# wwang2/CoarseGrainingVAE

Measured on NVIDIA B200. Metric: conformations/s (fwd+bwd train step), higher is better.
Workload: dtype f32

## Files before the change

coarsegrainingvae_b200/_lib.py:

```python
import ctypes
import os
import re

_HERE = os.path.dirname(os.path.abspath(__file__))
LIB_PATH = os.path.join(_HERE, "libcgvae_sm100.so")
HEADER_PATH = os.path.join(_HERE, "..", "include", "cgvae_b200.h")

_lib = None

_P = ctypes.c_void_p
_I64 = ctypes.c_int64
_INT = ctypes.c_int
_F32 = ctypes.c_float
_SZ = ctypes.c_size_t

SIGNATURES = {
    "cgvae_abi_version": (_INT, []),
    "cgvae_last_error": (ctypes.c_char_p, []),
    "cgvae_launch_count": (ctypes.c_ulonglong, []),
    "cgvae_set_error_flags": (_INT, [_INT, _P]),
    "cgvae_radius_graph_ws_bytes": (_SZ, [_I64, _I64]),
    "cgvae_radius_graph_count": (_INT, [_P, _I64, _P, _I64, _F32, _INT, _INT, _P, _P, _SZ, _P]),
    "cgvae_radius_graph_fill": (_INT, [_P, _I64, _P, _I64, _F32, _INT, _INT, _P, _P, _P, _SZ, _P]),
    "cgvae_exclusive_scan": (_INT, [_P, _I64, _P, _P]),
    "cgvae_edge_orientation": (_INT, [_P, _I64, _P, _P]),
    "cgvae_csr_count": (_INT, [_P, _I64, _P, _INT, _I64, _I64, _P, _P, _P]),
    "cgvae_scan_i32": (_INT, [_P, _I64, _P, _P]),
    "cgvae_csr_fill": (_INT, [_P, _I64, _P, _INT, _I64, _I64, _P, _P, _P, _P, _P, _P, _P, _P]),
    "cgvae_segment_count": (_INT, [_P, _I64, _I64, _P, _P]),
    "cgvae_segment_rank": (_INT, [_P, _I64, _I64, _P, _P, _P, _P, _P, _P]),
    "cgvae_edge_geometry": (_INT, [_P, _P, _P, _P, _P, _I64, _I64, _P, _INT, _INT, _F32, _P, _P, _P, _P, _P]),
    "cgvae_gemm": (_INT, [_INT, _P, _I64, _P, _I64, _P, _I64, _I64, _I64, _I64, _P, _INT, _P, _P, _INT, _P, _P, _SZ, _P, _INT, _P]),
    "cgvae_dense_pair_fwd": (_INT, [_P, _I64, _P, _I64, _I64, _I64, _I64, _I64, _P, _P, _P]),
    "cgvae_colsum": (_INT, [_P, _I64, _I64, _I64, _P, _P]),
    "cgvae_wgrad_grouped": (_INT, [_P, _INT, _P]),
    "cgvae_message_fwd": (_INT, [_INT, _P, _P, _P, _P, _P, _P, _P, _P, _P, _I64, _I64, _INT, _INT, _INT, _P, _P, _INT,
                                 _P, _P, _P, _P]),
    "cgvae_message_bwd_ws_bytes": (_SZ, [_INT, _INT, _INT, _I64]),
    "cgvae_message_bwd": (_INT, [_INT, _P, _P, _P, _P, _P, _P, _P, _P, _P, _P, _P, _I64, _I64, _INT, _INT, _INT, _P, _P,
                                 _INT, _INT, _P, _P, _P, _P, _P, _SZ, _P]),
    "cgvae_msg_tiles_batches_cap": (_I64, [_I64, _I64, _I64, _INT]),
    "cgvae_msg_tiles_rec_bytes": (_SZ, []),
    "cgvae_msg_tiles_build": (_INT, [_P, _P, _P, _I64, _I64, _I64, _P, _P, _INT, _INT, _P, _P, _P, _P, _I64, _P]),
    "cgvae_message_tc_ws_bytes": (_SZ, [_INT, _INT, _I64, _INT]),
    "cgvae_message_tc_fwd": (_INT, [_INT, _P, _P, _P, _P, _P, _P, _I64, _INT, _P, _P, _I64, _INT, _INT, _P, _P, _INT, _P, _P, _P,
                                    _P, _SZ, _P]),
    "cgvae_message9_fwd": (_INT, [_P, _P, _P, _P, _P, _P, _P, _P, _P, _P, _P, _I64, _INT, _INT, _INT, _INT, _P, _P, _P, _P, _P]),
    "cgvae_message9_bwd": (_INT, [_P, _P, _P, _P, _P, _P, _P, _P, _P, _P, _P, _P, _P, _P, _I64, _I64, _INT, _INT, _INT, _INT,
                                  _P, _P, _P, _P, _P, _P, _P, _P, _P, _P, _P]),
    "cgvae_update_norm_fwd": (_INT, [_P, _P, _I64, _INT, _P, _P]),
    "cgvae_update_combine_fwd": (_INT, [_P, _P, _P, _P, _P, _I64, _INT, _INT, _P, _P, _P]),
    "cgvae_update_combine_bwd": (_INT, [_P, _P, _P, _P, _P, _I64, _INT, _P, _P, _P, _P]),
    "cgvae_update_norm_bwd": (_INT, [_P, _P, _P, _P, _I64, _INT, _INT, _P, _P, _P]),
    "cgvae_update_combine_bwd_ld": (_INT, [_P, _P, _P, _P, _P, _I64, _INT, _P, _P, _P, _I64, _P]),
    "cgvae_update_norm_bwd_ld": (_INT, [_P, _P, _P, _P, _I64, _INT, _INT, _P, _P, _I64, _P]),
    "cgvae_segment_reduce_fwd": (_INT, [_P, _P, _P, _I64, _I64, _INT, _P, _P]),
    "cgvae_segment_reduce_bwd": (_INT, [_P, _P, _P, _I64, _I64, _INT, _P, _P]),
    "cgvae_gather_rows": (_INT, [_P, _P, _I64, _I64, _I64, _P, _P]),
    "cgvae_lift_fwd": (_INT, [_P, _P, _P, _P, _P, _P, _P, _I64, _I64, _INT, _INT, _P, _P]),
    "cgvae_lift_bwd": (_INT, [_P, _P, _P, _P, _P, _P, _I64, _I64, _INT, _INT, _P, _P]),
    "cgvae_adam_ws_bytes": (_SZ, []),
    "cgvae_adam_clip_step": (_INT, [_P, _P, _P, _P, _I64, _F32, _F32, _F32, _F32, _F32, _F32, _P, _P, _P, _F32, _F32, _P,
                                    _P, _SZ, _P]),
    "cgvae_bond_graph": (_INT, [_P, _P, _I64, _F32, _P, _P]),
    "cgvae_sample_quality": (_INT, [_P, _P, _P, _P, _I64, _I64, _F32, _P, _P, _P]),
    "cgvae_set_pdl": (_INT, [_INT]),
    "cgvae_set_matmul_precision": (_INT, [_INT]),
    "cgvae_get_matmul_precision": (_INT, []),
    "cgvae_register_const_range": (_INT, [_P, _SZ]),
    "cgvae_grad_sumsq": (_INT, [_P, _I64, _P, _P, _SZ, _P]),
    "cgvae_adam_apply": (_INT, [_P, _P, _P, _P, _I64, _F32, _F32, _F32, _F32, _F32, _F32, _P, _P, _INT, _F32, _F32, _P, _P, _SZ, _P]),
    "cgvae_dihedral_loss_fwd": (_INT, [_P, _P, _P, _I64, _P, _P, _P, _P, _P, _SZ, _P]),
    "cgvae_dihedral_loss_bwd": (_INT, [_P, _P, _P, _P, _I64, _I64, _P, _P, _P, _P]),
    "cgvae_pin_mask": (_INT, [_P, _I64, _P, _I64, _P, _SZ, _P]),
    "cgvae_vae_latent_fwd": (_INT, [_P, _P, _P, _I64, _P, _P, _P]),
    "cgvae_vae_latent_bwd": (_INT, [_P, _P, _P, _P, _I64, _P, _P, _P]),
    "cgvae_std_logvar_fwd": (_INT, [_P, _I64, _F32, _P, _P]),
    "cgvae_std_logvar_bwd": (_INT, [_P, _P, _I64, _F32, _P, _P]),
    "cgvae_loss_ws_bytes": (_SZ, []),
    "cgvae_loss_fwd": (_INT, [_P, _P, _I64, _P, _P, _P, _P, _P, _P, _I64, _INT, _P, _F32, _F32, _P, _P, _SZ, _P]),
    "cgvae_loss_bwd": (_INT, [_P, _P, _P, _I64, _P, _P, _P, _P, _P, _P, _I64, _INT, _P, _F32, _F32, _P, _P, _P, _P, _P, _P]),
    "cgvae_fill": (_INT, [_P, _I64, _F32, _P]),
    "cgvae_vec_to_planar": (_INT, [_P, _I64, _INT, _P, _P]),
    "cgvae_vec_from_planar": (_INT, [_P, _I64, _INT, _P, _P]),
}


def header_symbols():
    with open(HEADER_PATH) as fh:
        text = fh.read()
    text = re.sub(r"/\*.*?\*/", "", text, flags=re.S)
    return sorted(set(re.findall(r"\b(cgvae_[a-z0-9_]+)\s*\(", text)))


def load():
    global _lib
    if _lib is not None:
        return _lib
    if not os.path.exists(LIB_PATH):
        raise RuntimeError(
            "libcgvae_sm100.so not built (%s): run `python -m coarsegrainingvae_b200.build`; "
            "there is no CPU or PyTorch fallback" % LIB_PATH)
    lib = ctypes.CDLL(LIB_PATH)
    for name, (res, args) in SIGNATURES.items():
        fn = getattr(lib, name)
        fn.restype = res
        fn.argtypes = args
    if lib.cgvae_abi_version() != 1:
        raise RuntimeError("libcgvae_sm100.so ABI version mismatch")
    _lib = lib
    return lib


def last_error():
    return load().cgvae_last_error().decode("utf-8", "replace")


def launch_count():
    return int(load().cgvae_launch_count())


def check(rc, what):
    if rc != 0:
        raise RuntimeError("%s failed (code %d): %s" % (what, rc, last_error()))
```

coarsegrainingvae_b200/csrc/gemm_stream.cu:

```cuda
#include "common.cuh"
#include <cooperative_groups.h>
#include <cuda.h>
#include <algorithm>
#include <vector>

namespace cgvae {

struct StreamEpilogue {
  const float* bias;
  int act;
  float* z_out;
  const float* z_in;
  int dact;
  const float* add;
  float* C2;
  int n_split;
  int64_t ldc2;
};

__device__ __forceinline__ float stream_epilogue(const StreamEpilogue& ep, float v, int64_t m, int64_t n, int64_t ldc) {
  if (ep.bias) v += ep.bias[n];
  if (ep.z_out) ep.z_out[m * ldc + n] = v;
  v = act_fwd(ep.act, v);
  if (ep.z_in) v *= act_bwd(ep.dact, ep.z_in[m * ldc + n]);
  if (ep.add) v += ep.add[m * ldc + n];
  return v;
}

__host__ __device__ constexpr int wtr_count(int n, int off) { return (off >= 1 && n % 2 == 0) ? wtr_count(n / 2, off / 2) : n; }
__host__ __device__ constexpr int wtr_dupmask(int n, int off) { return (off >= 1 && n % 2 == 0) ? wtr_dupmask(n / 2, off / 2) : (off >= 1 ? 2 * off - 1 : 0); }

template <int N, int OFF>
__device__ __forceinline__ void wtr_step(float* v, int lane, int& base) {
  if constexpr (OFF >= 1 && (N % 2 == 0)) {
    constexpr int H = N / 2;
    const bool up = (lane & OFF) != 0;
#pragma unroll
    for (int i = 0; i < H; ++i) {
      const float send = up ? v[i] : v[i + H];
      const float keep = up ? v[i + H] : v[i];
      v[i] = keep + __shfl_xor_sync(0xffffffffu, send, OFF);
    }
    if (up) base += H;
    wtr_step<H, OFF / 2>(v, lane, base);
  } else if constexpr (OFF >= 1) {
#pragma unroll
    for (int i = 0; i < N; ++i) {
#pragma unroll
      for (int o = OFF; o >= 1; o >>= 1) v[i] += __shfl_xor_sync(0xffffffffu, v[i], o);
    }
  }
}

__device__ __forceinline__ uint32_t sm_u32(const void* p) { return (uint32_t)__cvta_generic_to_shared(p); }
__device__ __forceinline__ void bar_init(uint64_t* bar, uint32_t count) {
  asm volatile("mbarrier.init.shared::cta.b64 [%0], %1;" ::"r"(sm_u32(bar)), "r"(count));
}
__device__ __forceinline__ void bar_fence_init() { asm volatile("fence.mbarrier_init.release.cluster;" ::: "memory"); }
__device__ __forceinline__ void bar_expect_tx(uint64_t* bar, uint32_t bytes) {
  asm volatile("mbarrier.arrive.expect_tx.shared::cta.b64 _, [%0], %1;" ::"r"(sm_u32(bar)), "r"(bytes) : "memory");
}
__device__ __forceinline__ void bar_wait(uint64_t* bar, uint32_t parity) {
  for (uint32_t spin = 0; spin < (1u << 26); ++spin) {
    uint32_t done;
    asm volatile(
        "{\n"
        ".reg .pred p;\n"
        "mbarrier.try_wait.parity.shared::cta.b64 p, [%1], %2;\n"
        "selp.u32 %0, 1, 0, p;\n"
        "}\n"
        : "=r"(done)
        : "r"(sm_u32(bar)), "r"(parity)
        : "memory");
    if (done) return;
  }
  asm volatile("trap;");
}
__device__ __forceinline__ bool elect_lane() {
  uint32_t pred = 0;
  asm volatile(
      "{\n"
      ".reg .pred p;\n"
      "elect.sync _|p, 0xffffffff;\n"
      "selp.u32 %0, 1, 0, p;\n"
      "}\n"
      : "=r"(pred));
  return pred != 0;
}
__device__ __forceinline__ void bulk_g2s(void* dst, const void* src, uint32_t bytes, uint64_t* bar) {
  asm volatile("cp.async.bulk.shared::cluster.global.mbarrier::complete_tx::bytes [%0], [%1], %2, [%3];" ::"r"(sm_u32(dst)),
               "l"(src), "r"(bytes), "r"(sm_u32(bar))
               : "memory");
}
__device__ __forceinline__ void tma_2d_g2s(void* dst, const CUtensorMap* map, int c0, int c1, uint64_t* bar) {
  asm volatile("cp.async.bulk.tensor.2d.shared::cluster.global.mbarrier::complete_tx::bytes [%0], [%1, {%2, %3}], [%4];" ::"r"(
                   sm_u32(dst)),
               "l"(reinterpret_cast<uint64_t>(map)), "r"(c0), "r"(c1), "r"(sm_u32(bar))
               : "memory");
}

constexpr uint32_t kBulkPiece = 32768;

template <int MR, int RW>
__global__ void __launch_bounds__(MR > 16 ? 256 : 512) gemm_nt_stream_kernel(
    const float* __restrict__ X, int64_t ldx, const float* __restrict__ W, int64_t ldw, float* __restrict__ C, int64_t ldc,
    int M, int N, int K, int rows_per_cta, StreamEpilogue ep, int w_const) {
  if (!w_const) CGVAE_KERNEL_PROLOGUE();
  extern __shared__ __align__(128) float smem[];
  constexpr int NV = RW * MR;
  float* Xs = smem;
  float* Ws = smem + (size_t)MR * K;
  uint64_t* bar = reinterpret_cast<uint64_t*>(Ws + (size_t)rows_per_cta * K);
  const int tid = threadIdx.x, lane = tid & 31, warp = tid >> 5, nwarps = blockDim.x >> 5;
  const int row0 = blockIdx.x * rows_per_cta;
  const int rows = min(rows_per_cta, N - row0);

  if (tid == 0) {
    bar_init(bar, 1);
    bar_fence_init();
  }
  for (int idx = tid; idx < (MR - M) * (K / 4); idx += blockDim.x)
    reinterpret_cast<float4*>(Xs + (size_t)M * K)[idx] = make_float4(0.f, 0.f, 0.f, 0.f);
  __syncthreads();
  if (warp == 0 && elect_lane()) {
    const uint32_t row_bytes = (uint32_t)K * 4u;
    bar_expect_tx(bar, (uint32_t)(M + rows) * row_bytes);
    if (ldw == K) {
      const char* src = reinterpret_cast<const char*>(W + (int64_t)row0 * ldw);
      char* dst = reinterpret_cast<char*>(Ws);
      for (uint32_t off = 0, total = (uint32_t)rows * row_bytes; off < total; off += kBulkPiece)
        bulk_g2s(dst + off, src + off, min(kBulkPiece, total - off), bar);
    } else {
      for (int r = 0; r < rows; ++r) bulk_g2s(Ws + (size_t)r * K, W + (int64_t)(row0 + r) * ldw, row_bytes, bar);
    }
    if (w_const) pdl_wait();
    if (ldx == K) {
      const char* src = reinterpret_cast<const char*>(X);
      char* dst = reinterpret_cast<char*>(Xs);
      for (uint32_t off = 0, total = (uint32_t)M * row_bytes; off < total; off += kBulkPiece)
        bulk_g2s(dst + off, src + off, min(kBulkPiece, total - off), bar);
    } else {
      for (int m = 0; m < M; ++m) bulk_g2s(Xs + (size_t)m * K, X + (int64_t)m * ldx, row_bytes, bar);
    }
  }
  if (w_const) CGVAE_KERNEL_PROLOGUE();
  bar_wait(bar, 0);

  const int nchunks = (K + 127) / 128;
  for (int t0 = warp * RW; t0 < rows; t0 += nwarps * RW) {
    float acc[NV];
#pragma unroll
    for (int i = 0; i < NV; ++i) acc[i] = 0.f;
    for (int c = 0; c < nchunks; ++c) {
      const int k = c * 128 + lane * 4;
      if (k < K) {
        float4 w[RW];
#pragma unroll
        for (int r = 0; r < RW; ++r)
          w[r] = (t0 + r < rows) ? *reinterpret_cast<const float4*>(Ws + (size_t)(t0 + r) * K + k) : make_float4(0.f, 0.f, 0.f, 0.f);
#pragma unroll
        for (int m = 0; m < MR; ++m) {
          const float4 xv = *reinterpret_cast<const float4*>(Xs + (size_t)m * K + k);
#pragma unroll
          for (int r = 0; r < RW; ++r) {
            float a = acc[r * MR + m];
            a = fmaf(w[r].x, xv.x, a);
            a = fmaf(w[r].y, xv.y, a);
            a = fmaf(w[r].z, xv.z, a);
            a = fmaf(w[r].w, xv.w, a);
            acc[r * MR + m] = a;
          }
        }
      }
    }
    int base = 0;
    wtr_step<NV, 16>(acc, lane, base);
    constexpr int CNT = wtr_count(NV, 16);
    constexpr int DUP = wtr_dupmask(NV, 16);
    if ((lane & DUP) == 0) {
#pragma unroll
      for (int i = 0; i < CNT; ++i) {
        const int idx = base + i;
        const int r = idx / MR, m = idx % MR;
        const int n = row0 + t0 + r;
        if (m < M && t0 + r < rows) {
          if (ep.C2 != nullptr && n >= ep.n_split) ep.C2[(int64_t)m * ep.ldc2 + (n - ep.n_split)] = acc[i];
          else C[(int64_t)m * ldc + n] = stream_epilogue(ep, acc[i], m, n, ldc);
        }
      }
    }
  }
}

constexpr int NN_MAXBOX = 8;

template <int VEC> struct VecT;
template <> struct VecT<2> { using type = float2; };
template <> struct VecT<4> { using type = float4; };

template <int MR, int VEC, int NW>
__global__ void __launch_bounds__(NW * 32) gemm_nn_stream_kernel(
    const __grid_constant__ CUtensorMap wmap, const float* __restrict__ G, int64_t ldg, float* __restrict__ C, int64_t ldc,
    int M, int N, int K, int k_per_cta, int box_rows, StreamEpilogue ep, int w_const) {
  if (!w_const) CGVAE_KERNEL_PROLOGUE();
  namespace cg = cooperative_groups;
  using vec_t = typename VecT<VEC>::type;
  constexpr int COLS = 32 * VEC;
  extern __shared__ __align__(128) float smem[];
  const int nbox = (k_per_cta + box_rows - 1) / box_rows;
  float* Wt = smem;
  float* red = smem;
  const size_t wt_floats = (size_t)max(nbox * box_rows, NW * MR) * COLS;
  float* part = smem + wt_floats;
  float* Gt = part + MR * COLS;
  uint64_t* bars = reinterpret_cast<uint64_t*>(Gt + (size_t)k_per_cta * MR);
  const int tid = threadIdx.x, lane = tid & 31, warp = tid >> 5;
  const int col0 = blockIdx.x * COLS;
  const int kbeg = blockIdx.z * k_per_cta;
  const int cnt = max(0, min(K, kbeg + k_per_cta) - kbeg);

  if (tid == 0) {
    for (int b = 0; b < nbox; ++b) bar_init(bars + b, 1);
    bar_fence_init();
  }
  __syncwarp();
  if (warp == 0 && elect_lane()) {
    for (int b = 0; b < nbox; ++b) {
      if (b * box_rows < cnt) {
        bar_expect_tx(bars + b, (uint32_t)box_rows * COLS * 4u);
        tma_2d_g2s(Wt + (size_t)b * box_rows * COLS, &wmap, col0, kbeg + b * box_rows, bars + b);
      }
    }
  }
  if (w_const) CGVAE_KERNEL_PROLOGUE();
  for (int idx = tid; idx < MR * cnt; idx += NW * 32) {
    const int m = idx / cnt, j = idx - m * cnt;
    Gt[j * MR + m] = (m < M) ? __ldg(G + (int64_t)m * ldg + kbeg + j) : 0.f;
  }
  __syncthreads();

  float acc[MR][VEC];
#pragma unroll
  for (int m = 0; m < MR; ++m)
#pragma unroll
    for (int v = 0; v < VEC; ++v) acc[m][v] = 0.f;

  for (int b = 0; b * box_rows < cnt; ++b) {
    bar_wait(bars + b, 0);
    const int jend = min(cnt, (b + 1) * box_rows);
#pragma unroll 2
    for (int j = b * box_rows + warp; j < jend; j += NW) {
      const vec_t t = *reinterpret_cast<const vec_t*>(Wt + (size_t)j * COLS + lane * VEC);
      float w[VEC];
      if constexpr (VEC == 2) { w[0] = t.x; w[1] = t.y; }
      if constexpr (VEC == 4) { w[0] = t.x; w[1] = t.y; w[2] = t.z; w[3] = t.w; }
      const float* g = Gt + j * MR;
#pragma unroll
      for (int m4 = 0; m4 < MR / 4; ++m4) {
        const float4 g4 = *reinterpret_cast<const float4*>(g + 4 * m4);
#pragma unroll
        for (int v = 0; v < VEC; ++v) {
          acc[4 * m4 + 0][v] = fmaf(g4.x, w[v], acc[4 * m4 + 0][v]);
          acc[4 * m4 + 1][v] = fmaf(g4.y, w[v], acc[4 * m4 + 1][v]);
          acc[4 * m4 + 2][v] = fmaf(g4.z, w[v], acc[4 * m4 + 2][v]);
          acc[4 * m4 + 3][v] = fmaf(g4.w, w[v], acc[4 * m4 + 3][v]);
        }
      }
    }
  }
  __syncthreads();
#pragma unroll
  for (int m = 0; m < MR; ++m)
#pragma unroll
    for (int v = 0; v < VEC; ++v) red[(warp * MR + m) * COLS + lane * VEC + v] = acc[m][v];
  __syncthreads();
  for (int o = tid; o < MR * COLS; o += NW * 32) {
    float s = 0.f;
#pragma unroll
    for (int wv = 0; wv < NW; ++wv) s += red[wv * MR * COLS + o];
    part[o] = s;
  }
  cg::cluster_group cluster = cg::this_cluster();
  cluster.sync();
  const int S = (int)cluster.num_blocks(), rank = (int)cluster.block_rank();
  for (int o = tid; o < MR * COLS; o += NW * 32) {
    const int m = o / COLS, c = o - m * COLS;
    if (m % S != rank) continue;
    const int n = col0 + c;
    if (m < M && n < N) {
      float s = 0.f;
      for (int z = 0; z < S; ++z) s += *cluster.map_shared_rank(part + o, z);
      C[(int64_t)m * ldc + n] = stream_epilogue(ep, s, m, n, ldc);
    }
  }
  cluster.sync();
}

typedef CUresult (*EncodeTiledFn)(CUtensorMap*, CUtensorMapDataType, cuuint32_t, void*, const cuuint64_t*, const cuuint64_t*,
                                  const cuuint32_t*, const cuuint32_t*, CUtensorMapInterleave, CUtensorMapSwizzle,
                                  CUtensorMapL2promotion, CUtensorMapFloatOOBfill);

static EncodeTiledFn encode_tiled_fn() {
  static EncodeTiledFn fn = [] {
    void* p = nullptr;
    cudaDriverEntryPointQueryResult q;
    if (cudaGetDriverEntryPoint("cuTensorMapEncodeTiled", &p, cudaEnableDefault, &q) != cudaSuccess || q != cudaDriverEntryPointSuccess) {
      (void)cudaGetLastError();
      p = nullptr;
    }
    return reinterpret_cast<EncodeTiledFn>(p);
  }();
  return fn;
}

constexpr size_t kMaxStreamSmem = 220 * 1024;

struct ConstRange {
  uintptr_t begin, end;
};
static std::vector<ConstRange> g_const_ranges;

bool weights_are_constant(const void* p, size_t bytes) {
  if (!pdl_enabled() || g_const_ranges.empty()) return false;
  const uintptr_t a = reinterpret_cast<uintptr_t>(p);
  auto it = std::upper_bound(g_const_ranges.begin(), g_const_ranges.end(), a,
                             [](uintptr_t v, const ConstRange& r) { return v < r.begin; });
  if (it == g_const_ranges.begin()) return false;
  --it;
  return a >= it->begin && a + bytes <= it->end;
}

template <int MR, int RW>
static bool launch_nt(const float* X, int64_t ldx, const float* W, int64_t ldw, float* C, int64_t ldc, int M, int N, int K,
                      const StreamEpilogue& ep, cudaStream_t st) {
  const int w_const = weights_are_constant(W, sizeof(float) * ((size_t)(N - 1) * (size_t)ldw + (size_t)K)) ? 1 : 0;
  int rpc = (int)ceil_div(ceil_div(N, kNumSM), RW) * RW;
  const size_t smem = sizeof(float) * ((size_t)MR * K + (size_t)rpc * K) + 16;
  if (smem > kMaxStreamSmem) return false;
  static size_t attr_bytes = 0;
  if (smem > attr_bytes) {
    if (cudaFuncSetAttribute(gemm_nt_stream_kernel<MR, RW>, cudaFuncAttributeMaxDynamicSharedMemorySize, (int)kMaxStreamSmem) != cudaSuccess) {
      (void)cudaGetLastError();
      return false;
    }
    attr_bytes = kMaxStreamSmem;
  }
  const int tasks = rpc / RW;
  const int nwarps = tasks <= 2 ? 2 : (tasks <= 4 ? 4 : ((tasks <= 8 || MR > 16) ? 8 : 16));
  launch_kernel(gemm_nt_stream_kernel<MR, RW>, dim3((unsigned)ceil_div(N, rpc)), dim3(nwarps * 32), smem, st, X, ldx, W, ldw, C, ldc, M,
                N, K, rpc, ep, w_const);
  return true;
}

template <int MR, int VEC, int NW>
static bool launch_nn(const float* G, int64_t ldg, const float* W, int64_t ldw, float* C, int64_t ldc, int M, int N, int K,
                      const StreamEpilogue& ep, cudaStream_t st) {
  const int w_const = weights_are_constant(W, sizeof(float) * ((size_t)(K - 1) * (size_t)ldw + (size_t)N)) ? 1 : 0;
  constexpr int COLS = 32 * VEC;
  EncodeTiledFn encode = encode_tiled_fn();
  if (encode == nullptr) return false;
  const int blocks = (int)ceil_div(N, COLS);
  int S = (int)std::min<int64_t>(8, std::max<int64_t>(1, kNumSM / blocks));
  S = (int)std::min<int64_t>(S, std::max<int64_t>(1, K / NW));
  while (S & (S - 1)) S &= S - 1;
  int k_per_cta = (int)ceil_div(K, S);
  S = (int)ceil_div(K, k_per_cta);
  const int nbox = (int)ceil_div(k_per_cta, 256);
  if (nbox > NN_MAXBOX) return false;
  const int box_rows = (int)ceil_div(k_per_cta, nbox);
  const size_t wt_floats = (size_t)std::max(nbox * box_rows, NW * MR) * COLS;
  const size_t smem = sizeof(float) * (wt_floats + (size_t)MR * COLS + (size_t)k_per_cta * MR) + 8 * NN_MAXBOX;
  if (smem > kMaxStreamSmem) return false;
  CUtensorMap map;
  const cuuint64_t gdim[2] = {(cuuint64_t)N, (cuuint64_t)K};
  const cuuint64_t gstride[1] = {(cuuint64_t)ldw * 4};
  const cuuint32_t box[2] = {(cuuint32_t)COLS, (cuuint32_t)box_rows};
  const cuuint32_t estride[2] = {1, 1};
  if (encode(&map, CU_TENSOR_MAP_DATA_TYPE_FLOAT32, 2, const_cast<float*>(W), gdim, gstride, box, estride, CU_TENSOR_MAP_INTERLEAVE_NONE,
             CU_TENSOR_MAP_SWIZZLE_NONE, CU_TENSOR_MAP_L2_PROMOTION_L2_256B, CU_TENSOR_MAP_FLOAT_OOB_FILL_NONE) != CUDA_SUCCESS)
    return false;
  static size_t attr_bytes = 0;
  if (smem > attr_bytes) {
    if (cudaFuncSetAttribute(gemm_nn_stream_kernel<MR, VEC, NW>, cudaFuncAttributeMaxDynamicSharedMemorySize, (int)kMaxStreamSmem) != cudaSuccess) {
      (void)cudaGetLastError();
      return false;
    }
    attr_bytes = kMaxStreamSmem;
  }
  cudaLaunchConfig_t cfg = {};
  cfg.gridDim = dim3((unsigned)blocks, 1, (unsigned)S);
  cfg.blockDim = dim3(NW * 32);
  cfg.dynamicSmemBytes = smem;
  cfg.stream = st;
  cudaLaunchAttribute attr[2];
  attr[0].id = cudaLaunchAttributeClusterDimension;
  attr[0].val.clusterDim.x = 1;
  attr[0].val.clusterDim.y = 1;
  attr[0].val.clusterDim.z = (unsigned)S;
  attr[1].id = cudaLaunchAttributeProgrammaticStreamSerialization;
  attr[1].val.programmaticStreamSerializationAllowed = 1;
  cfg.attrs = attr;
  cfg.numAttrs = pdl_enabled() ? 2 : 1;
  (void)cudaLaunchKernelEx(&cfg, gemm_nn_stream_kernel<MR, VEC, NW>, map, G, ldg, C, ldc, M, N, K, k_per_cta, box_rows, ep, w_const);
  return true;
}

int launch_gemm_stream(int form, const float* A, int64_t lda, const float* B, int64_t ldb, float* C, int64_t ldc, int64_t M,
                       int64_t N, int64_t K, const float* bias, int act, float* z_out, const float* z_in, int dact,
                       const float* add, cudaStream_t st) {
  static const bool enabled = [] { const char* e = getenv("CGVAE_STREAM_GEMM"); return !(e && e[0] == '0'); }();
  if (!enabled || M > 48 || M < 1 || form == CGVAE_GEMM_TN) return 0;
  if (N * K < 64 * 64 || N >= (1 << 24) || K >= (1 << 24)) return 0;
  const StreamEpilogue ep{bias, act, z_out, z_in, dact, add, nullptr, 0, 0};
  const int m = (int)M, n = (int)N, k = (int)K;
  if (form == CGVAE_GEMM_NT) {
    if (K % 4 != 0 || K < 128 || lda % 4 != 0 || ldb % 4 != 0 || !aligned16(A) || !aligned16(B)) return 0;
    if (M <= 12) return launch_nt<12, 4>(A, lda, B, ldb, C, ldc, m, n, k, ep, st);
    if (M <= 16) return launch_nt<16, 4>(A, lda, B, ldb, C, ldc, m, n, k, ep, st);
    if (M <= 36) return launch_nt<36, 2>(A, lda, B, ldb, C, ldc, m, n, k, ep, st);
    return launch_nt<48, 2>(A, lda, B, ldb, C, ldc, m, n, k, ep, st);
  }
  if (K < 64 || N < 64 || ldb % 4 != 0 || !aligned16(B)) return 0;
  const bool wide = ceil_div(N, 64) * 2 > kNumSM;
  if (M <= 12) return wide ? launch_nn<12, 4, 16>(A, lda, B, ldb, C, ldc, m, n, k, ep, st) : launch_nn<12, 2, 16>(A, lda, B, ldb, C, ldc, m, n, k, ep, st);
  if (M <= 16) return wide ? launch_nn<16, 4, 16>(A, lda, B, ldb, C, ldc, m, n, k, ep, st) : launch_nn<16, 2, 16>(A, lda, B, ldb, C, ldc, m, n, k, ep, st);
  static const bool nn_wide_rows = [] { const char* e = getenv("CGVAE_STREAM_NN_ROWS48"); return e && e[0] == '1'; }();
  if (!nn_wide_rows) return 0;
  if (M <= 36) return launch_nn<36, 2, 8>(A, lda, B, ldb, C, ldc, m, n, k, ep, st);
  return launch_nn<48, 2, 8>(A, lda, B, ldb, C, ldc, m, n, k, ep, st);
}

int launch_dense_pair_stream(const float* X, int64_t ldx, const float* W, int64_t ldw, float* C1, int64_t ldc1, float* C2,
                             int64_t ldc2, int64_t M, int64_t N1, int64_t N2, int64_t K, cudaStream_t st) {
  static const bool enabled = [] { const char* e = getenv("CGVAE_STREAM_GEMM"); return !(e && e[0] == '0'); }();
  if (!enabled || M > 48 || M < 1 || N1 + N2 >= (1 << 24) || K >= (1 << 24)) return 0;
  if (K % 4 != 0 || K < 128 || ldx % 4 != 0 || ldw % 4 != 0 || !aligned16(X) || !aligned16(W)) return 0;
  const StreamEpilogue ep{nullptr, 0, nullptr, nullptr, 0, nullptr, C2, (int)N1, ldc2};
  const int m = (int)M, n = (int)(N1 + N2), k = (int)K;
  if (M <= 12) return launch_nt<12, 4>(X, ldx, W, ldw, C1, ldc1, m, n, k, ep, st);
  if (M <= 16) return launch_nt<16, 4>(X, ldx, W, ldw, C1, ldc1, m, n, k, ep, st);
  if (M <= 36) return launch_nt<36, 2>(X, ldx, W, ldw, C1, ldc1, m, n, k, ep, st);
  return launch_nt<48, 2>(X, ldx, W, ldw, C1, ldc1, m, n, k, ep, st);
}

}

extern "C" {

int cgvae_register_const_range(const void* p, size_t bytes) {
  using namespace cgvae;
  if (p == nullptr || bytes == 0) {
    g_const_ranges.clear();
    return 0;
  }
  ConstRange r{reinterpret_cast<uintptr_t>(p), reinterpret_cast<uintptr_t>(p) + bytes};
  std::vector<ConstRange> out;
  out.reserve(g_const_ranges.size() + 1);
  for (const ConstRange& q : g_const_ranges) {
    if (q.end < r.begin || q.begin > r.end) out.push_back(q);
    else {
      r.begin = std::min(r.begin, q.begin);
      r.end = std::max(r.end, q.end);
    }
  }
  out.push_back(r);
  std::sort(out.begin(), out.end(), [](const ConstRange& x, const ConstRange& y) { return x.begin < y.begin; });
  g_const_ranges.swap(out);
  return 0;
}

}
```

coarsegrainingvae_b200/csrc/nodewise.cu:

```cuda
#include "common.cuh"

namespace cgvae {

__global__ void __launch_bounds__(256) update_norm_fwd_kernel(const float* __restrict__ s, const float* __restrict__ Vv, int64_t N,
                                                              int F, float* __restrict__ x) {
  CGVAE_KERNEL_PROLOGUE();
  const int64_t idx = (int64_t)blockIdx.x * blockDim.x + threadIdx.x;
  if (idx >= N * F) return;
  const int64_t n = idx / F;
  const int f = (int)(idx % F);
  const float* p = Vv + n * 3 * F + f;
  const float a = __fadd_rn(__fmul_rn(p[0], p[0]), 1e-10f);
  const float b = __fadd_rn(__fmul_rn(p[F], p[F]), 1e-10f);
  const float c = __fadd_rn(__fmul_rn(p[2 * (int64_t)F], p[2 * (int64_t)F]), 1e-10f);
  x[n * 2 * F + f] = s[idx];
  x[n * 2 * F + F + f] = __fsqrt_rn(__fadd_rn(__fadd_rn(a, b), c));
}

__global__ void __launch_bounds__(256) update_combine_fwd_kernel(const float* __restrict__ s, const float* __restrict__ v,
                                                                 const float* __restrict__ Uv, const float* __restrict__ Vv,
                                                                 const float* __restrict__ q, int64_t N, int F, int residual,
                                                                 float* __restrict__ s_out, float* __restrict__ v_out) {
  CGVAE_KERNEL_PROLOGUE();
  const int64_t idx = (int64_t)blockIdx.x * blockDim.x + threadIdx.x;
  if (idx >= N * F) return;
  const int64_t n = idx / F;
  const int f = (int)(idx % F);
  const int64_t o = n * 3 * F + f;
  const float a_vv = q[o], a_sv = q[o + F], a_ss = q[o + 2 * (int64_t)F];
  float inner = 0.f;
#pragma unroll
  for (int c = 0; c < 3; ++c) {
    const float u = Uv[o + (int64_t)c * F], w = Vv[o + (int64_t)c * F];
    inner = fmaf(u, w, inner);
    v_out[o + (int64_t)c * F] = (residual ? v[o + (int64_t)c * F] : 0.f) + u * a_vv;
  }
  s_out[idx] = (residual ? s[idx] : 0.f) + (inner * a_sv + a_ss);
}

__global__ void __launch_bounds__(256) update_combine_bwd_kernel(const float* __restrict__ Uv, const float* __restrict__ Vv,
                                                                 const float* __restrict__ q, const float* __restrict__ g_s,
                                                                 const float* __restrict__ g_v, int64_t N, int F,
                                                                 float* __restrict__ gq, float* __restrict__ gUv,
                                                                 float* __restrict__ gVv, int64_t ldg) {
  CGVAE_KERNEL_PROLOGUE();
  const int64_t idx = (int64_t)blockIdx.x * blockDim.x + threadIdx.x;
  if (idx >= N * F) return;
  const int64_t n = idx / F;
  const int f = (int)(idx % F);
  const int64_t o = n * 3 * F + f;
  const int64_t og = n * 3 * ldg + f;
  const float a_vv = q[o], a_sv = q[o + F];
  const float gs = g_s[idx];
  float inner = 0.f, g_avv = 0.f;
  const float t = gs * a_sv;
#pragma unroll
  for (int c = 0; c < 3; ++c) {
    const float u = Uv[o + (int64_t)c * F], w = Vv[o + (int64_t)c * F], g = g_v[o + (int64_t)c * F];
    inner = fmaf(u, w, inner);
    g_avv = fmaf(g, u, g_avv);
    gUv[og + (int64_t)c * ldg] = g * a_vv + t * w;
    gVv[og + (int64_t)c * ldg] = t * u;
  }
  gq[o] = g_avv;
  gq[o + F] = gs * inner;
  gq[o + 2 * (int64_t)F] = gs;
}

__global__ void __launch_bounds__(256) update_norm_bwd_kernel(const float* __restrict__ x, const float* __restrict__ Vv,
                                                              const float* __restrict__ gx, const float* __restrict__ g_s,
                                                              int64_t N, int F, int residual, float* __restrict__ gs_in,
                                                              float* __restrict__ gVv, int64_t ldg) {
  CGVAE_KERNEL_PROLOGUE();
  const int64_t idx = (int64_t)blockIdx.x * blockDim.x + threadIdx.x;
  if (idx >= N * F) return;
  const int64_t n = idx / F;
  const int f = (int)(idx % F);
  gs_in[idx] = (residual ? g_s[idx] : 0.f) + gx[n * 2 * F + f];
  const float scale = gx[n * 2 * F + F + f] / x[n * 2 * F + F + f];
  const int64_t o = n * 3 * F + f, og = n * 3 * ldg + f;
#pragma unroll
  for (int c = 0; c < 3; ++c) gVv[og + (int64_t)c * ldg] = fmaf(scale, Vv[o + (int64_t)c * F], gVv[og + (int64_t)c * ldg]);
}

__global__ void __launch_bounds__(256) segment_reduce_fwd_kernel(const float* __restrict__ X, const int32_t* __restrict__ rowptr_b,
                                                                 const int32_t* __restrict__ atoms, int64_t W, int mean,
                                                                 float* __restrict__ out) {
  CGVAE_KERNEL_PROLOGUE();
  const int64_t b = blockIdx.x;
  const int64_t w = (int64_t)blockIdx.y * blockDim.x + threadIdx.x;
  if (w >= W) return;
  const int beg = rowptr_b[b], end = rowptr_b[b + 1];
  float acc = 0.f;
  for (int t = beg; t < end; ++t) acc += X[(int64_t)atoms[t] * W + w];
  if (mean) acc = acc / (float)max(end - beg, 1);
  out[b * W + w] = acc;
}
__global__ void __launch_bounds__(256) segment_reduce_bwd_kernel(const float* __restrict__ g_out, const int64_t* __restrict__ mapping,
                                                                 const int32_t* __restrict__ rowptr_b, int64_t W, int mean,
                                                                 float* __restrict__ g_X) {
  CGVAE_KERNEL_PROLOGUE();
  const int64_t a = blockIdx.x;
  const int64_t w = (int64_t)blockIdx.y * blockDim.x + threadIdx.x;
  if (w >= W) return;
  const int64_t b = mapping[a];
  float g = g_out[b * W + w];
  if (mean) g = g / (float)max(rowptr_b[b + 1] - rowptr_b[b], 1);
  g_X[a * W + w] = g;
}

__global__ void __launch_bounds__(256) gather_rows_kernel(const float* __restrict__ table, const int64_t* __restrict__ idx, int64_t W,
                                                          int64_t n_rows, float* __restrict__ out, int32_t* __restrict__ err) {
  CGVAE_KERNEL_PROLOGUE();
  const int64_t n = blockIdx.x;
  const int64_t w = (int64_t)blockIdx.y * blockDim.x + threadIdx.x;
  if (w >= W) return;
  const int64_t r = idx[n];
  if (n_rows > 0 && (r < 0 || r >= n_rows)) {
    if (w == 0) raise_flag(err, CGVAE_ERR_EMBED_INDEX);
    out[n * W + w] = __int_as_float(0x7fc00000);
    return;
  }
  out[n * W + w] = table[r * W + w];
}

__global__ void __launch_bounds__(128) lift_fwd_kernel(const float* __restrict__ V, const float* __restrict__ cg_xyz,
                                                       const int64_t* __restrict__ rank, const int32_t* __restrict__ rowptr_b,
                                                       const int32_t* __restrict__ atoms, const uint8_t* __restrict__ pin,
                                                       int64_t n_beads, int F, int mode, float* __restrict__ xyz_out,
                                                       int32_t* __restrict__ err) {
  CGVAE_KERNEL_PROLOGUE();
  const int lane = threadIdx.x & 31;
  const int64_t b = (int64_t)blockIdx.x * 4 + (threadIdx.x >> 5);
  if (b >= n_beads) return;
  const int beg = rowptr_b[b], end = rowptr_b[b + 1];
  const float* Vb = V + b * 3 * F;
  float mean[3] = {0.f, 0.f, 0.f};
  if (mode == 1) {
    for (int t = beg + lane; t < end; t += 32) {
      const int64_t ch = rank[atoms[t]];
      if (ch >= F) continue;
#pragma unroll
      for (int c = 0; c < 3; ++c) mean[c] += Vb[(int64_t)c * F + ch];
    }
    const float inv = 1.0f / (float)max(end - beg, 1);
#pragma unroll
    for (int c = 0; c < 3; ++c) mean[c] = warp_sum(mean[c]) * inv;
  }
  for (int t = beg + lane; t < end; t += 32) {
    const int a = atoms[t];
    const int64_t ch = rank[a];
    const bool pinned = (mode == 2) && pin != nullptr && pin[a] != 0;
    if (ch >= F) {
      raise_flag(err, CGVAE_ERR_LIFT_RANK);
#pragma unroll
      for (int c = 0; c < 3; ++c) xyz_out[(int64_t)a * 3 + c] = __int_as_float(0x7fc00000);
      continue;
    }
#pragma unroll
    for (int c = 0; c < 3; ++c) {
      const float rel = pinned ? 0.f : Vb[(int64_t)c * F + ch] - mean[c];
      xyz_out[(int64_t)a * 3 + c] = rel + cg_xyz[b * 3 + c];
    }
  }
}
__global__ void __launch_bounds__(128) lift_bwd_kernel(const float* __restrict__ g_xyz, const int64_t* __restrict__ rank,
                                                       const int32_t* __restrict__ rowptr_b, const int32_t* __restrict__ atoms,
                                                       const uint8_t* __restrict__ pin, int64_t n_beads, int F, int mode,
                                                       float* __restrict__ g_V) {
  CGVAE_KERNEL_PROLOGUE();
  const int lane = threadIdx.x & 31;
  const int64_t b = (int64_t)blockIdx.x * 4 + (threadIdx.x >> 5);
  if (b >= n_beads) return;
  const int beg = rowptr_b[b], end = rowptr_b[b + 1];
  float* gVb = g_V + b * 3 * F;
  float mean[3] = {0.f, 0.f, 0.f};
  if (mode == 1) {
    for (int t = beg + lane; t < end; t += 32) {
      const int a = atoms[t];
#pragma unroll
      for (int c = 0; c < 3; ++c) mean[c] += g_xyz[(int64_t)a * 3 + c];
    }
    const float inv = 1.0f / (float)max(end - beg, 1);
#pragma unroll
    for (int c = 0; c < 3; ++c) mean[c] = warp_sum(mean[c]) * inv;
  }
  for (int t = beg + lane; t < end; t += 32) {
    const int a = atoms[t];
    const int64_t ch = rank[a];
    const bool pinned = (mode == 2) && pin != nullptr && pin[a] != 0;
    if (ch >= F) continue;
#pragma unroll
    for (int c = 0; c < 3; ++c) gVb[(int64_t)c * F + ch] = pinned ? 0.f : g_xyz[(int64_t)a * 3 + c] - mean[c];
  }
}

__global__ void __launch_bounds__(256) pin_mask_kernel(const int64_t* __restrict__ idx, int64_t n_idx, const int64_t* __restrict__ n_live,
                                                       int64_t n_atoms, uint8_t* __restrict__ pin, int32_t* __restrict__ err) {
  CGVAE_KERNEL_PROLOGUE();
  const int64_t n = n_live ? min(*n_live, n_idx) : n_idx;
  const int64_t i = (int64_t)blockIdx.x * blockDim.x + threadIdx.x;
  if (i >= n || n <= 0) return;
  if (idx[n - 1] >= n_atoms) return;
  const int64_t a = idx[i];
  if (a < 0 || a >= n_atoms) {
    raise_flag(err, CGVAE_ERR_NODE_INDEX);
    return;
  }
  pin[a] = 1;
}

}

using namespace cgvae;

extern "C" {

int cgvae_pin_mask(const int64_t* idx, int64_t n_idx, const int64_t* n_live, int64_t n_atoms, uint8_t* pin, size_t pin_bytes,
                   cgvae_stream_t stream) {
  cudaStream_t st = (cudaStream_t)stream;
  if (n_atoms == 0) return 0;
  CGVAE_REQUIRE(pin && pin_bytes >= (size_t)n_atoms && pin_bytes % 4 == 0, "pin_mask: pin buffer must hold n_atoms bytes, padded to 4");
  CGVAE_ZERO(pin, pin_bytes, st);
  if (n_idx == 0) return 0;
  CGVAE_REQUIRE(idx, "pin_mask: null index list");
  launch_kernel(pin_mask_kernel, dim3((unsigned)ceil_div(n_idx, 256)), dim3(256), 0, st, idx, n_idx, n_live, n_atoms, pin, err_flags());
  return launched("pin_mask");
}

int cgvae_update_norm_fwd(const float* s, const float* Vv, int64_t N, int F, float* x, cgvae_stream_t stream) {
  if (N == 0) return 0;
  CGVAE_REQUIRE(s && Vv && x, "update_norm_fwd: null pointer");
  launch_kernel(update_norm_fwd_kernel, dim3((unsigned)ceil_div(N * F, 256)), dim3(256), 0, (cudaStream_t)stream, s, Vv, N, F, x);
  return launched("update_norm_fwd");
}
int cgvae_update_combine_fwd(const float* s, const float* v, const float* Uv, const float* Vv, const float* q, int64_t N, int F,
                             int residual, float* s_out, float* v_out, cgvae_stream_t stream) {
  if (N == 0) return 0;
  CGVAE_REQUIRE(Uv && Vv && q && s_out && v_out && (!residual || (s && v)), "update_combine_fwd: null pointer");
  launch_kernel(update_combine_fwd_kernel, dim3((unsigned)ceil_div(N * F, 256)), dim3(256), 0, (cudaStream_t)stream, s, v, Uv, Vv, q, N, F, residual, s_out,
                                                                                             v_out);
  return launched("update_combine_fwd");
}
int cgvae_update_combine_bwd(const float* Uv, const float* Vv, const float* q, const float* g_s, const float* g_v, int64_t N, int F,
                             float* gq, float* gUv, float* gVv, cgvae_stream_t stream) {
  if (N == 0) return 0;
  CGVAE_REQUIRE(Uv && Vv && q && g_s && g_v && gq && gUv && gVv, "update_combine_bwd: null pointer");
  launch_kernel(update_combine_bwd_kernel, dim3((unsigned)ceil_div(N * F, 256)), dim3(256), 0, (cudaStream_t)stream, Uv, Vv, q, g_s, g_v, N, F, gq, gUv, gVv, (int64_t)F);
  return launched("update_combine_bwd");
}
int cgvae_update_norm_bwd(const float* x, const float* Vv, const float* gx, const float* g_s, int64_t N, int F, int residual,
                          float* gs_in, float* gVv, cgvae_stream_t stream) {
  if (N == 0) return 0;
  CGVAE_REQUIRE(x && Vv && gx && gs_in && gVv && (!residual || g_s), "update_norm_bwd: null pointer");
  launch_kernel(update_norm_bwd_kernel, dim3((unsigned)ceil_div(N * F, 256)), dim3(256), 0, (cudaStream_t)stream, x, Vv, gx, g_s, N, F, residual, gs_in, gVv, (int64_t)F);
  return launched("update_norm_bwd");
}

int cgvae_update_combine_bwd_ld(const float* Uv, const float* Vv, const float* q, const float* g_s, const float* g_v, int64_t N, int F,
                                float* gq, float* gUv, float* gVv, int64_t ldg, cgvae_stream_t stream) {
  if (N == 0) return 0;
  CGVAE_REQUIRE(Uv && Vv && q && g_s && g_v && gq && gUv && gVv && ldg >= F, "update_combine_bwd_ld: bad arguments");
  launch_kernel(update_combine_bwd_kernel, dim3((unsigned)ceil_div(N * F, 256)), dim3(256), 0, (cudaStream_t)stream, Uv, Vv, q, g_s, g_v, N, F, gq,
                gUv, gVv, ldg);
  return launched("update_combine_bwd");
}
int cgvae_update_norm_bwd_ld(const float* x, const float* Vv, const float* gx, const float* g_s, int64_t N, int F, int residual,
                             float* gs_in, float* gVv, int64_t ldg, cgvae_stream_t stream) {
  if (N == 0) return 0;
  CGVAE_REQUIRE(x && Vv && gx && gs_in && gVv && (!residual || g_s) && ldg >= F, "update_norm_bwd_ld: bad arguments");
  launch_kernel(update_norm_bwd_kernel, dim3((unsigned)ceil_div(N * F, 256)), dim3(256), 0, (cudaStream_t)stream, x, Vv, gx, g_s, N, F, residual,
                gs_in, gVv, ldg);
  return launched("update_norm_bwd");
}

int cgvae_segment_reduce_fwd(const float* X, const int32_t* rowptr_b, const int32_t* atoms, int64_t n_beads, int64_t W, int mean,
                             float* out, cgvae_stream_t stream) {
  if (n_beads == 0 || W == 0) return 0;
  CGVAE_REQUIRE(X && rowptr_b && atoms && out, "segment_reduce_fwd: null pointer");
  dim3 grid((unsigned)n_beads, (unsigned)ceil_div(W, 256));
  launch_kernel(segment_reduce_fwd_kernel, dim3(grid), dim3(256), 0, (cudaStream_t)stream, X, rowptr_b, atoms, W, mean, out);
  return launched("segment_reduce_fwd");
}
int cgvae_segment_reduce_bwd(const float* g_out, const int64_t* mapping, const int32_t* rowptr_b, int64_t N, int64_t W, int mean,
                             float* g_X, cgvae_stream_t stream) {
  if (N == 0 || W == 0) return 0;
  CGVAE_REQUIRE(g_out && mapping && rowptr_b && g_X, "segment_reduce_bwd: null pointer");
  dim3 grid((unsigned)N, (unsigned)ceil_div(W, 256));
  launch_kernel(segment_reduce_bwd_kernel, dim3(grid), dim3(256), 0, (cudaStream_t)stream, g_out, mapping, rowptr_b, W, mean, g_X);
  return launched("segment_reduce_bwd");
}
int cgvae_gather_rows(const float* table, const int64_t* idx, int64_t N, int64_t W, int64_t n_rows, float* out,
                      cgvae_stream_t stream) {
  if (N == 0 || W == 0) return 0;
  CGVAE_REQUIRE(table && idx && out, "gather_rows: null pointer");
  dim3 grid((unsigned)N, (unsigned)ceil_div(W, 256));
  launch_kernel(gather_rows_kernel, dim3(grid), dim3(256), 0, (cudaStream_t)stream, table, idx, W, n_rows, out, err_flags());
  return launched("gather_rows");
}

int cgvae_lift_fwd(const float* V, const float* cg_xyz, const int64_t* mapping, const int64_t* rank, const int32_t* rowptr_b,
                   const int32_t* atoms, const uint8_t* pin, int64_t N, int64_t n_beads, int F, int mode, float* xyz_out,
                   cgvae_stream_t stream) {
  (void)mapping;
  if (N == 0 || n_beads == 0) return 0;
  CGVAE_REQUIRE(V && cg_xyz && rank && rowptr_b && atoms && xyz_out, "lift_fwd: null pointer");
  CGVAE_REQUIRE(mode >= 0 && mode <= 2, "lift_fwd: bad mode %d", mode);
  launch_kernel(lift_fwd_kernel, dim3((unsigned)ceil_div(n_beads, 4)), dim3(128), 0, (cudaStream_t)stream, V, cg_xyz, rank, rowptr_b, atoms, pin, n_beads, F,
                                                                                   mode, xyz_out, err_flags());
  return launched("lift_fwd");
}
int cgvae_lift_bwd(const float* g_xyz, const int64_t* mapping, const int64_t* rank, const int32_t* rowptr_b, const int32_t* atoms,
                   const uint8_t* pin, int64_t N, int64_t n_beads, int F, int mode, float* g_V, cgvae_stream_t stream) {
  (void)mapping;
  cudaStream_t st = (cudaStream_t)stream;
  if (n_beads == 0) return 0;
  CGVAE_REQUIRE(g_xyz && rank && rowptr_b && atoms && g_V, "lift_bwd: null pointer");
  CGVAE_ZERO(g_V, sizeof(float) * (size_t)n_beads * 3 * (size_t)F, st);
  if (N == 0) return 0;
  launch_kernel(lift_bwd_kernel, dim3((unsigned)ceil_div(n_beads, 4)), dim3(128), 0, st, g_xyz, rank, rowptr_b, atoms, pin, n_beads, F, mode, g_V);
  return launched("lift_bwd");
}

}
```

coarsegrainingvae_b200/functions.py:

```python
import torch
from torch.autograd import Function
from torch.autograd.function import once_differentiable

from . import ops

SWISH = 1


def _phi_forward(s, W1, b1, W2, b2, act=SWISH):
    a1, z1 = ops.linear_fwd(s, W1, b1, act, save_pre=True)
    phi = ops.linear_fwd(a1, W2, b2, 0)
    return a1, z1, phi


def _phi_backward(g_phi2d, s, a1, z1, W1, b1, W2, b2, add_to_gs, act=SWISH):
    fork = ops.Fork(g_phi2d.device, enabled=not ops.deferring(g_phi2d.shape[0]))
    gz1 = ops.linear_bwd_input(g_phi2d, W2, z_in=z1, dact=act)
    with fork.branch():
        gW2 = ops.linear_bwd_weight(g_phi2d, a1, W2)
        gb2 = ops.colsum(g_phi2d, b2)
    fork.sync()
    gs = ops.linear_bwd_input(gz1, W1, add=add_to_gs)
    with fork.branch():
        gW1 = ops.linear_bwd_weight(gz1, s, W1)
        gb1 = ops.colsum(gz1, b1)
    fork.join()
    return gs, gW1, gb1, gW2, gb2


class MLP2(Function):

    @staticmethod
    def forward(ctx, act, x, W1, b1, W2, b2):
        x = x.contiguous()
        a1, z1, y = _phi_forward(x, W1, b1, W2, b2, act)
        ctx.act = act
        ctx.save_for_backward(x, a1, z1, W1, b1, W2, b2)
        return y

    @staticmethod
    @once_differentiable
    def backward(ctx, gy):
        x, a1, z1, W1, b1, W2, b2 = ctx.saved_tensors
        gx, gW1, gb1, gW2, gb2 = _phi_backward(gy.contiguous(), x, a1, z1, W1, b1, W2, b2, None, ctx.act)
        return None, gx, gW1, gb1, gW2, gb2


class LinearFn(Function):

    @staticmethod
    def forward(ctx, x, W, b):
        x = x.contiguous()
        ctx.save_for_backward(x, W, b)
        return ops.linear_fwd(x, W, b, 0)

    @staticmethod
    @once_differentiable
    def backward(ctx, gy):
        x, W, b = ctx.saved_tensors
        gy = gy.contiguous()
        fork = ops.Fork(gy.device, enabled=not ops.deferring(gy.shape[0]))
        gx = ops.linear_bwd_input(gy, W)
        with fork.branch():
            gW = ops.linear_bwd_weight(gy, x, W)
            gb = ops.colsum(gy, b) if b is not None else None
        fork.join()
        return gx, gW, gb


class MessageBlock(Function):

    @staticmethod
    def forward(ctx, geom, n_split, mode, act, s, v, res_s, res_v, W1, b1, W2, b2, Wf, bf):
        s = s.contiguous()
        a1, z1, phi = _phi_forward(s, W1, b1, W2, b2, act)
        N, F = s.shape
        phi3 = phi.view(N, n_split, F)
        if mode == "self":
            rs, rv = s, v
        elif mode == "other":
            rs, rv = res_s, res_v
        else:
            rs, rv = None, None
        out_s, out_v, q = ops.message_fwd(n_split, phi3, v, v if n_split == 4 else None, geom, Wf, bf, rs, rv,
                                          want_q=(n_split == 4 and v is not None))
        ctx.geom, ctx.n_split, ctx.mode, ctx.act = geom, n_split, mode, act
        ctx.v_none = v is None
        ctx.res_v_none = res_v is None
        ctx.save_for_backward(s, v, a1, z1, phi3, q, W1, b1, W2, b2, Wf, bf)
        return out_s, out_v

    @staticmethod
    @once_differentiable
    def backward(ctx, g_s, g_v):
        s, v, a1, z1, phi3, q, W1, b1, W2, b2, Wf, bf = ctx.saved_tensors
        g_s, g_v = g_s.contiguous(), g_v.contiguous()
        n_split, mode = ctx.n_split, ctx.mode
        residual = mode == "self"
        g_phi, g_v_send, dWf, dbf = ops.message_bwd(n_split, phi3, v, v if n_split == 4 else None, q, ctx.geom, Wf, bf,
                                                    g_s, g_v, residual and not ctx.v_none)
        N, F = s.shape
        gs, gW1, gb1, gW2, gb2 = _phi_backward(g_phi.view(N, n_split * F), s, a1, z1, W1, b1, W2, b2,
                                               g_s if residual else None, ctx.act)
        gv = None if ctx.v_none else g_v_send
        g_res_s = g_s if mode == "other" else None
        g_res_v = g_v if (mode == "other" and not ctx.res_v_none) else None
        return None, None, None, None, gs, gv, g_res_s, g_res_v, gW1, gb1, gW2, gb2, dWf, dbf


class Message9Block(Function):

    @staticmethod
    def forward(ctx, geom, residual, act, s, sbar, v, vbar, W1, b1, W2, b2, Wf, bf):
        s, sbar, v, vbar = s.contiguous(), sbar.contiguous(), v.contiguous(), vbar.contiguous()
        a1, z1, phi = _phi_forward(s, W1, b1, W2, b2, act)
        N, F = s.shape
        phi3 = phi.view(N, 9, F)
        outs = ops.message9_fwd(phi3, s, sbar, v, vbar, geom, Wf, bf, residual)
        ctx.geom, ctx.residual, ctx.act = geom, residual, act
        ctx.save_for_backward(s, sbar, v, vbar, a1, z1, phi3, W1, b1, W2, b2, Wf, bf)
        return tuple(outs)

    @staticmethod
    @once_differentiable
    def backward(ctx, g_s, g_sbar, g_v, g_vbar):
        s, sbar, v, vbar, a1, z1, phi3, W1, b1, W2, b2, Wf, bf = ctx.saved_tensors
        gi_s, gi_sbar, gi_v, gi_vbar, g_phi, dWf, dbf = ops.message9_bwd(
            phi3, s, sbar, v, vbar, ctx.geom, Wf, bf, ctx.residual,
            g_s.contiguous(), g_sbar.contiguous(), g_v.contiguous(), g_vbar.contiguous())
        N, F = s.shape
        gs, gW1, gb1, gW2, gb2 = _phi_backward(g_phi.view(N, 9 * F), s, a1, z1, W1, b1, W2, b2, gi_s, ctx.act)
        return None, None, None, gs, gi_sbar, gi_v, gi_vbar, gW1, gb1, gW2, gb2, dWf, dbf


class UpdateBlockFn(Function):

    @staticmethod
    def forward(ctx, residual, act, s, v, U, V, A0, c0, A1, c1):
        s, v = s.contiguous(), v.contiguous()
        N, F = s.shape
        v2 = v.view(3 * N, F)
        Uv, Vv = ops.linear_pair_fwd(v2, U, V)
        Uv, Vv = Uv.view(N, 3, F), Vv.view(N, 3, F)
        x = ops.update_norm_fwd(s, Vv)
        h, z = ops.linear_fwd(x, A0, c0, act, save_pre=True)
        q = ops.linear_fwd(h, A1, c1, 0).view(N, 3, F)
        s_out, v_out = ops.update_combine_fwd(s, v, Uv, Vv, q, residual)
        ctx.residual, ctx.act = residual, act
        ctx.save_for_backward(v, Uv, Vv, x, h, z, q, U, V, A0, c0, A1, c1)
        return s_out, v_out

    @staticmethod
    @once_differentiable
    def backward(ctx, g_s, g_v):
        v, Uv, Vv, x, h, z, q, U, V, A0, c0, A1, c1 = ctx.saved_tensors
        g_s, g_v = g_s.contiguous(), g_v.contiguous()
        N, _, F = v.shape
        pair = (U.is_cuda and U.is_contiguous() and V.is_contiguous() and U.shape == V.shape
                and V.data_ptr() == U.data_ptr() + 4 * U.numel()
                and U.untyped_storage().data_ptr() == V.untyped_storage().data_ptr())
        gq, gUv, gVv = ops.update_combine_bwd(Uv, Vv, q, g_s, g_v, cat=pair)
        gq2 = gq.view(N, 3 * F)
        v2 = v.view(3 * N, F)
        if pair:
            gUV2 = gUv.as_strided((3 * N, 2 * F), (2 * F, 1))
            gUv2, gVv2 = gUV2[:, :F], gUV2[:, F:]
        else:
            gUv2, gVv2 = gUv.view(3 * N, F), gVv.view(3 * N, F)
        fork = ops.Fork(g_s.device, enabled=not ops.deferring(3 * N))
        gz = ops.linear_bwd_input(gq2, A1, z_in=z, dact=ctx.act)
        with fork.branch():
            gA1 = ops.linear_bwd_weight(gq2, h, A1)
            gc1 = ops.colsum(gq2, c1)
            if not pair:
                gU = ops.linear_bwd_weight(gUv2, v2, U)
        fork.sync()
        gx = ops.linear_bwd_input(gz, A0)
        with fork.branch():
            gA0 = ops.linear_bwd_weight(gz, x, A0)
            gc0 = ops.colsum(gz, c0)
        gs_in = ops.update_norm_bwd(x, Vv, gx, g_s, gVv, ctx.residual)
        fork.sync()
        if pair:
            UV = U.as_strided((2 * F, U.shape[1]), (U.shape[1], 1))
            gv_in = ops.linear_bwd_input(gUV2, UV, add=g_v.view(3 * N, F) if ctx.residual else None).view(N, 3, F)
        else:
            gv_in = ops.linear_bwd_input(gUv2, U, add=g_v.view(3 * N, F) if ctx.residual else None)
            gv_in = ops.linear_bwd_input(gVv2, V, add=gv_in).view(N, 3, F)
        with fork.branch():
            if pair:
                gUVw = ops.linear_bwd_weight(gUV2, v2, U, shape=(2 * F, U.shape[1]))
                gU, gV = gUVw[:F], gUVw[F:]
            else:
                gV = ops.linear_bwd_weight(gVv2, v2, V)
        fork.join()
        return None, None, gs_in, gv_in, gU, gV, gA0, gc0, gA1, gc1


class SegmentReduce(Function):

    @staticmethod
    def forward(ctx, seg, mean, X):
        ctx.seg, ctx.mean = seg, mean
        return ops.segment_reduce_fwd(X.contiguous(), seg, mean)

    @staticmethod
    @once_differentiable
    def backward(ctx, g):
        return None, None, ops.segment_reduce_bwd(g.contiguous(), ctx.seg, ctx.mean)


class EmbeddingLookup(Function):

    @staticmethod
    def forward(ctx, table, idx, padding_idx):
        idx = idx.to(torch.int64).contiguous()
        ctx.padding_idx = padding_idx
        ctx.n_rows = table.shape[0]
        ctx.save_for_backward(idx, table)
        return ops.gather_rows(table, idx)

    @staticmethod
    @once_differentiable
    def backward(ctx, g):
        idx, table = ctx.saved_tensors
        seg = ops.build_segments(idx, ctx.n_rows)
        gt = ops.segment_reduce_fwd(g.contiguous(), seg, False, param=table)
        if ctx.padding_idx is not None:
            gt[ctx.padding_idx].zero_()
        return gt, None, None


class Lift(Function):

    @staticmethod
    def forward(ctx, seg, mode, pin, V, cg_xyz):
        ctx.seg, ctx.mode, ctx.pin, ctx.F = seg, mode, pin, V.shape[-1]
        return ops.lift_fwd(V.contiguous(), cg_xyz, seg, mode, pin)

    @staticmethod
    @once_differentiable
    def backward(ctx, g):
        return None, None, None, ops.lift_bwd(g.contiguous(), ctx.seg, ctx.F, ctx.mode, ctx.pin), None


class VAELatent(Function):

    @staticmethod
    def forward(ctx, mu, logvar, eps):
        z, sigma = ops.vae_latent_fwd(mu, logvar, eps)
        ctx.save_for_backward(eps, sigma)
        return z, sigma

    @staticmethod
    @once_differentiable
    def backward(ctx, g_z, g_sigma):
        eps, sigma = ctx.saved_tensors
        g_mu, g_logvar = ops.vae_latent_bwd(g_z.contiguous() if g_z is not None else None,
                                            g_sigma.contiguous() if g_sigma is not None else None, eps, sigma)
        return g_mu, g_logvar, None


class StdLogvar(Function):

    @staticmethod
    def forward(ctx, x, c):
        y = ops.std_logvar_fwd(x, c)
        ctx.c = c
        ctx.save_for_backward(y)
        return y

    @staticmethod
    @once_differentiable
    def backward(ctx, gy):
        (y,) = ctx.saved_tensors
        return ops.std_logvar_bwd(gy.contiguous(), y, ctx.c), None


class TrainingLoss(Function):

    @staticmethod
    def forward(ctx, bond_graph, beta, gamma, norms, xyz, xyz_rec, mu, sigma, pmu, pstd):
        xyz, xyz_rec = xyz.contiguous(), xyz_rec.contiguous()
        if mu is not None:
            mu, sigma = mu.contiguous(), sigma.contiguous()
        if pmu is not None:
            pmu, pstd = pmu.contiguous(), pstd.contiguous()
        out4 = ops.loss_fwd(xyz, xyz_rec, bond_graph, mu, sigma, pmu, pstd, norms, beta, gamma)
        ctx.bond_graph, ctx.beta, ctx.gamma, ctx.norms = bond_graph, beta, gamma, norms
        ctx.has = (mu is not None, pmu is not None)
        ctx.save_for_backward(xyz, xyz_rec, *([mu, sigma] if mu is not None else []), *([pmu, pstd] if pmu is not None else []))
        comps = out4.detach()
        ctx.mark_non_differentiable(comps)
        return out4.narrow(0, 0, 1).reshape(()), comps

    @staticmethod
    @once_differentiable
    def backward(ctx, g_loss, _g_comps):
        saved = list(ctx.saved_tensors)
        xyz, xyz_rec = saved[0], saved[1]
        mu = sigma = pmu = pstd = None
        k = 2
        if ctx.has[0]:
            mu, sigma = saved[k], saved[k + 1]
            k += 2
        if ctx.has[1]:
            pmu, pstd = saved[k], saved[k + 1]
        g = g_loss.reshape(1).contiguous()
        g_rec, g_mu, g_sigma, g_pmu, g_pstd = ops.loss_bwd(g, xyz, xyz_rec, ctx.bond_graph, mu, sigma, pmu, pstd, ctx.norms,
                                                           ctx.beta, ctx.gamma)
        return None, None, None, None, None, g_rec, g_mu, g_sigma, g_pmu, g_pstd


class DihedralLoss(Function):

    @staticmethod
    def forward(ctx, xyz, xyz_rec, idx, count, norm):
        n_atoms = xyz_rec.shape[0]
        idx = idx.to(torch.int64).contiguous()
        out, contrib = ops.dihedral_loss_fwd(xyz.contiguous(), xyz_rec.contiguous(), idx, count, norm)
        D = idx.shape[0]
        pairs = torch.stack([idx.reshape(-1), torch.arange(4 * D, dtype=torch.int64, device=idx.device)], 1)
        ctx.graph = ops.build_graph(pairs, n_atoms, n_send=max(4 * D, 1))
        ctx.n_atoms, ctx.count, ctx.norm = n_atoms, count, norm
        ctx.save_for_backward(contrib)
        return out.reshape(())

    @staticmethod
    @once_differentiable
    def backward(ctx, g):
        (contrib,) = ctx.saved_tensors
        g_rec = ops.dihedral_loss_bwd(g.reshape(1).contiguous(), contrib, ctx.graph, ctx.n_atoms, ctx.count, ctx.norm)
        return None, g_rec, None, None, None
```

coarsegrainingvae_b200/ops.py:

```python
import contextlib as _contextlib

import numpy as np
import torch

from . import _lib

ACT_CODES = {None: 0, "none": 0, "linear": 0, "swish": 1, "ReLU": 2, "relu": 2, "Tanh": 3, "tanh": 3}
GEMM_NT, GEMM_NN, GEMM_TN = 0, 1, 2


def _p(t):
    if t is None:
        return None
    return t.data_ptr()


_raw_stream = torch._C._cuda_getCurrentRawStream if hasattr(torch._C, "_cuda_getCurrentRawStream") else None


def _stream():
    if _raw_stream is not None:
        return _raw_stream(torch.cuda.current_device())
    return torch.cuda.current_stream().cuda_stream


def _need_cuda(*tensors):
    for t in tensors:
        if t is not None and not t.is_cuda:
            raise RuntimeError("coarsegrainingvae_b200 runs on CUDA tensors only (sm_100a kernels, no CPU fallback); "
                               "got a %s tensor" % t.device)


def _f32(t):
    if t.dtype != torch.float32:
        raise RuntimeError("expected float32, got %s" % t.dtype)
    return t.contiguous()


def launch_count():
    return _lib.launch_count()


VALIDATE = True
_ERR_FLAGS = {}
_ERR_TEXT = {1: "a bead holds more atoms than feature channels (cg_v[mapping, CG2atomChannel], cgvae.py:473)",
             2: "embedding index out of range (nn.Embedding, cgvae.py:273,380,591)",
             4: "CG_mapping entry outside [0, n_beads)",
             8: "edge-list entry outside [0, n_nodes)"}


def error_flags(device):
    idx = device.index if device.index is not None else torch.cuda.current_device()
    t = _ERR_FLAGS.get(idx)
    if t is None:
        t = torch.zeros(1, dtype=torch.int32, device=torch.device("cuda", idx))
        _ERR_FLAGS[idx] = t
        _lib.check(_lib.load().cgvae_set_error_flags(idx, t.data_ptr()), "set_error_flags")
    return t


def check_device_errors(device, force=False):
    if not (VALIDATE or force) or device.type != "cuda" or torch.cuda.is_current_stream_capturing():
        return
    t = error_flags(device)
    bits = int(t.item())
    if bits:
        t.zero_()
        raise IndexError("; ".join(msg for bit, msg in _ERR_TEXT.items() if bits & bit))


class KernelTimer(object):

    def __init__(self, names, keep_operands=False):
        self.names = set(names)
        self.records = {}
        self.keep_operands = keep_operands

    def begin(self, name):
        if name not in self.names:
            return None
        ev = torch.cuda.Event(enable_timing=True)
        ev.record(torch.cuda.current_stream())
        return ev

    def end(self, name, start, meta):
        if start is None:
            return
        ev = torch.cuda.Event(enable_timing=True)
        ev.record(torch.cuda.current_stream())
        self.records.setdefault(name, []).append((start, ev, meta))

    def summary(self):
        return {k: [(a.elapsed_time(b), m) for a, b, m in v] for k, v in self.records.items()}


TIMER = None

_SIDE_STREAMS = {}
FORK_ENABLED = True


class Fork(object):

    def __init__(self, device, enabled=True):
        self.enabled = enabled and FORK_ENABLED and device.type == "cuda"
        if not self.enabled:
            return
        idx = device.index if device.index is not None else torch.cuda.current_device()
        side = _SIDE_STREAMS.get(idx)
        if side is None:
            side = torch.cuda.Stream(device=idx)
            _SIDE_STREAMS[idx] = side
        self.side = side
        self.main = torch.cuda.current_stream(idx)
        self.sync()

    def sync(self):
        if self.enabled:
            ev = torch.cuda.Event()
            ev.record(self.main)
            self.side.wait_event(ev)

    def branch(self):
        if self.enabled:
            return torch.cuda.stream(self.side)
        import contextlib
        return contextlib.nullcontext()

    def join(self):
        if self.enabled:
            ev = torch.cuda.Event()
            ev.record(self.side)
            self.main.wait_event(ev)


GRAD_SINK = {}


def _has_sink(param):
    return (param is not None and bool(GRAD_SINK) and param.grad is None and GRAD_SINK.get(param.data_ptr()) is not None)


def _grad_out(param, shape):
    hit = GRAD_SINK.get(param.data_ptr()) if GRAD_SINK else None
    if hit is None or param.grad is not None:
        return torch.empty(shape, dtype=param.dtype, device=param.device)
    flat, off = hit
    n = 1
    for s in shape:
        n *= s
    return flat[off:off + n].view(shape)



class Graph(object):

    def __init__(self, n_recv, n_send, n_edges, rowptr, col, eid, rowptr_t, col_t, perm_t):
        self.n_recv, self.n_send, self.n_edges = int(n_recv), int(n_send), int(n_edges)
        self.rowptr, self.col, self.eid = rowptr, col, eid
        self.rowptr_t, self.col_t, self.perm_t = rowptr_t, col_t, perm_t


class Geometry(object):

    def __init__(self, graph, basis, unit, n_rbf, rb, cutoff):
        self.graph, self.basis, self.unit = graph, basis, unit
        self.n_rbf, self.rb, self.cutoff = int(n_rbf), int(rb), float(cutoff)


class Segments(object):

    def __init__(self, n_beads, mapping, rowptr, atoms, slot, rank):
        self.n_beads, self.mapping = int(n_beads), mapping
        self.rowptr, self.atoms, self.slot, self.rank = rowptr, atoms, slot, rank
        self.n = int(mapping.shape[0])


def rb_for(n_rbf):
    rb = ((n_rbf + 1 + 3) // 4) * 4
    if rb < 8:
        rb = 8
    if rb > 16:
        raise RuntimeError("n_rbf up to 15 supported (got %d)" % n_rbf)
    return rb


_COEF_CACHE = {}


def rbf_coefficients(n_rbf, cutoff, device):
    key = (int(n_rbf), float(cutoff), str(device))
    hit = _COEF_CACHE.get(key)
    if hit is None:
        n = torch.arange(1, n_rbf + 1).float()
        hit = (n * np.pi / cutoff).to(device)
        _COEF_CACHE[key] = hit
    return hit


def exclusive_scan(counts_i32, out_dtype=torch.int64):
    _need_cuda(counts_i32)
    lib = _lib.load()
    n = counts_i32.shape[0]
    out = torch.empty(n + 1, dtype=out_dtype, device=counts_i32.device)
    if out_dtype == torch.int64:
        _lib.check(lib.cgvae_exclusive_scan(_p(counts_i32), n, _p(out), _stream()), "exclusive_scan")
    else:
        _lib.check(lib.cgvae_scan_i32(_p(counts_i32), n, _p(out), _stream()), "scan_i32")
    return out


def radius_graph(xyz, cutoff, undirected=True, frame_ptr=None, use_cells=None, capacity=None, max_frame=None):
    _need_cuda(xyz)
    lib = _lib.load()
    xyz = _f32(xyz)
    n = xyz.shape[0]
    dev = xyz.device
    if frame_ptr is None:
        frame_ptr = torch.tensor([0, n], dtype=torch.int64, device=dev)
        max_frame = n
    else:
        frame_ptr = frame_ptr.to(device=dev, dtype=torch.int64).contiguous()
    n_frames = frame_ptr.shape[0] - 1
    if capacity is not None:
        if max_frame is None:
            raise ValueError("radius_graph(capacity=...) needs max_frame (atoms of the largest frame): no host read in static mode")
        worst = n_frames * max_frame * (max_frame - 1) // (2 if undirected else 1)
        if capacity < worst:
            raise ValueError("capacity %d below the worst case %d (%d frames of <= %d atoms)" % (capacity, worst, n_frames, max_frame))
    if use_cells is None:
        if max_frame is None:
            max_frame = int((frame_ptr[1:] - frame_ptr[:-1]).max().item()) if n_frames > 0 else 0
        use_cells = max_frame > 1024
    if n == 0:
        if capacity is not None:
            return torch.zeros((capacity, 2), dtype=torch.int64, device=dev), torch.zeros(1, dtype=torch.int64, device=dev)
        return torch.zeros((0, 2), dtype=torch.int64, device=dev)
    ws_bytes = int(lib.cgvae_radius_graph_ws_bytes(n, n_frames)) if use_cells else 0
    ws = torch.empty(max(ws_bytes, 16), dtype=torch.uint8, device=dev)
    deg = torch.empty(n, dtype=torch.int32, device=dev)
    st = _stream()
    _lib.check(lib.cgvae_radius_graph_count(_p(xyz), n, _p(frame_ptr), n_frames, float(np.float32(cutoff)), int(bool(undirected)),
                                            int(bool(use_cells)), _p(deg), _p(ws), ws_bytes, st), "radius_graph_count")
    rowptr = exclusive_scan(deg, torch.int64)
    if capacity is not None:
        pairs = torch.zeros((capacity, 2), dtype=torch.int64, device=dev)
        _lib.check(lib.cgvae_radius_graph_fill(_p(xyz), n, _p(frame_ptr), n_frames, float(np.float32(cutoff)), int(bool(undirected)),
                                               int(bool(use_cells)), _p(rowptr), _p(pairs), _p(ws), ws_bytes, st),
                   "radius_graph_fill")
        return pairs, rowptr[-1:].clone()
    n_edges = int(rowptr[-1].item())
    pairs = torch.empty((n_edges, 2), dtype=torch.int64, device=dev)
    if n_edges:
        _lib.check(lib.cgvae_radius_graph_fill(_p(xyz), n, _p(frame_ptr), n_frames, float(np.float32(cutoff)), int(bool(undirected)),
                                               int(bool(use_cells)), _p(rowptr), _p(pairs), _p(ws), ws_bytes, st),
                   "radius_graph_fill")
    return pairs


def edge_orientation(pairs):
    _need_cuda(pairs)
    lib = _lib.load()
    flags = torch.empty(2, dtype=torch.int32, device=pairs.device)
    pairs = pairs.contiguous()
    _lib.check(lib.cgvae_edge_orientation(_p(pairs), pairs.shape[0], _p(flags), _stream()), "edge_orientation")
    f = flags.tolist()
    return bool(f[0]), bool(f[1])


def build_graph(pairs, n_recv, n_send=None, symmetrize=False, n_edges_dev=None):
    _need_cuda(pairs)
    lib = _lib.load()
    if n_send is None:
        n_send = n_recv
    pairs = pairs.to(torch.int64).contiguous()
    E_in = pairs.shape[0]
    E = 2 * E_in if symmetrize else E_in
    dev = pairs.device
    st = _stream()
    sym = int(bool(symmetrize))
    error_flags(dev)
    deg_r = torch.empty(n_recv, dtype=torch.int32, device=dev)
    deg_s = torch.empty(n_send, dtype=torch.int32, device=dev)
    _lib.check(lib.cgvae_csr_count(_p(pairs), E_in, _p(n_edges_dev), sym, n_recv, n_send, _p(deg_r), _p(deg_s), st), "csr_count")
    rowptr = exclusive_scan(deg_r, torch.int32)
    rowptr_t = exclusive_scan(deg_s, torch.int32)
    col = torch.empty(E, dtype=torch.int32, device=dev)
    eid = torch.empty(E, dtype=torch.int32, device=dev)
    col_t = torch.empty(E, dtype=torch.int32, device=dev)
    perm_t = torch.empty(E, dtype=torch.int32, device=dev)
    scratch = torch.empty(n_recv + n_send + 2 * E + 4, dtype=torch.int32, device=dev)
    _lib.check(lib.cgvae_csr_fill(_p(pairs), E_in, _p(n_edges_dev), sym, n_recv, n_send, _p(rowptr), _p(rowptr_t), _p(scratch),
                                  _p(col), _p(eid), _p(col_t), _p(perm_t), st), "csr_fill")
    return Graph(n_recv, n_send, E, rowptr, col, eid, rowptr_t, col_t, perm_t)


def build_segments(mapping, n_beads):
    _need_cuda(mapping)
    lib = _lib.load()
    mapping = mapping.to(torch.int64).contiguous()
    n = mapping.shape[0]
    dev = mapping.device
    st = _stream()
    error_flags(dev)
    deg = torch.empty(n_beads, dtype=torch.int32, device=dev)
    _lib.check(lib.cgvae_segment_count(_p(mapping), n, n_beads, _p(deg), st), "segment_count")
    rowptr = exclusive_scan(deg, torch.int32)
    atoms = torch.empty(n, dtype=torch.int32, device=dev)
    slot = torch.empty(n, dtype=torch.int32, device=dev)
    rank = torch.empty(n, dtype=torch.int64, device=dev)
    scratch = torch.empty(n_beads + 4, dtype=torch.int32, device=dev)
    _lib.check(lib.cgvae_segment_rank(_p(mapping), n, n_beads, _p(rowptr), _p(scratch), _p(atoms), _p(slot), _p(rank), st),
               "segment_rank")
    return Segments(n_beads, mapping, rowptr, atoms, slot, rank)


def contraction_graph(seg):
    dev = seg.mapping.device
    n = seg.n
    rowptr_t = torch.arange(n + 1, dtype=torch.int32, device=dev)
    col_t = seg.mapping.to(torch.int32)
    return Graph(seg.n_beads, n, n, seg.rowptr, seg.atoms, seg.atoms, rowptr_t, col_t, seg.slot)


def edge_geometry(graph, xyz_send, xyz_recv, n_rbf, cutoff, edge_wgt=None, r_edge=None):
    _need_cuda(xyz_send, xyz_recv, r_edge)
    lib = _lib.load()
    dev = (r_edge if r_edge is not None else xyz_send).device
    rb = rb_for(n_rbf)
    E = graph.n_edges
    basis = torch.empty((E, rb), dtype=torch.float32, device=dev)
    unit = torch.empty((E, 4), dtype=torch.float32, device=dev)
    coef = rbf_coefficients(n_rbf, cutoff, dev)
    xs = _f32(xyz_send) if xyz_send is not None else None
    xr = _f32(xyz_recv) if xyz_recv is not None else None
    re = _f32(r_edge) if r_edge is not None else None
    w = _f32(edge_wgt) if edge_wgt is not None else None
    _lib.check(lib.cgvae_edge_geometry(_p(xs), _p(xr), _p(re), _p(graph.rowptr), _p(graph.col), graph.n_recv, E, _p(coef), n_rbf, rb,
                                       float(np.float32(cutoff)), _p(w), _p(graph.eid), _p(basis), _p(unit), _stream()),
               "edge_geometry")
    return Geometry(graph, basis, unit, n_rbf, rb, cutoff)



_SPLITK_WS_BYTES = 32 << 20
_N_TICKETS = 1024
_TICKETS = {}


def _tickets(dev, stream):
    key = (dev.index, stream)
    t = _TICKETS.get(key)
    if t is None:
        t = torch.zeros(_N_TICKETS, dtype=torch.int32, device=dev)
        _TICKETS[key] = t
    return t


def gemm(form, A, B, M, N, K, bias=None, act=0, z_out=False, z_in=None, dact=0, add=None, out=None):
    _need_cuda(A, B)
    if A.dtype != torch.float32 or B.dtype != torch.float32 or A.stride(-1) != 1 or B.stride(-1) != 1:
        raise RuntimeError("gemm: operands must be float32 with unit inner stride (got %s %s, %s %s)"
                           % (A.dtype, tuple(A.stride()), B.dtype, tuple(B.stride())))
    lib = _lib.load()
    dev = A.device
    if out is not None and (out.dtype != torch.float32 or out.device != dev or tuple(out.shape) != (M, N)
                            or (N > 1 and out.stride(1) != 1)):
        raise RuntimeError("gemm: out must be a float32 (%d, %d) tensor with unit inner stride on %s (got %s %s %s on %s)"
                           % (M, N, dev, out.dtype, tuple(out.shape), tuple(out.stride()), out.device))
    C = out if out is not None else torch.empty((M, N), dtype=torch.float32, device=dev)
    ldc = C.stride(0)
    if bias is not None and (bias.dtype != torch.float32 or bias.dim() != 1 or bias.numel() != N
                             or not bias.is_contiguous() or bias.device != dev):
        raise RuntimeError("gemm: bias must be a contiguous float32 vector of length %d on %s (got %s %s %s on %s)"
                           % (N, dev, bias.dtype, tuple(bias.shape), tuple(bias.stride()), bias.device))
    for name, t in (("z_in", z_in), ("add", add)):
        if t is not None and (t.dtype != torch.float32 or tuple(t.shape) != (M, N) or (N > 1 and t.stride(1) != 1)
                              or (M > 1 and t.stride(0) != ldc) or t.device != dev):
            raise RuntimeError("gemm: %s must be a float32 (%d, %d) tensor on %s with the row stride of the output (%d) "
                               "and unit inner stride (got %s %s %s on %s)"
                               % (name, M, N, dev, ldc, t.dtype, tuple(t.shape), tuple(t.stride()), t.device))
    if z_out and M > 1 and ldc != N:
        raise RuntimeError("gemm: z_out=True needs an output with row stride %d (the pre-activation copy is a contiguous "
                           "(M, N) tensor indexed with the output's row stride); got row stride %d" % (N, ldc))
    Z = torch.empty((M, N), dtype=torch.float32, device=dev) if z_out else None
    tiles = ((M + 63) // 64) * ((N + 63) // 64) if M > 32 else ((N + 31) // 32)
    st = _stream()
    ws = tk = None
    if (tiles < 148 and K >= 512) or (K > 24576 and M >= 64):
        ws = torch.empty(_SPLITK_WS_BYTES, dtype=torch.uint8, device=dev)
        tk = _tickets(dev, st)
    t0 = TIMER.begin("gemm") if TIMER is not None else None
    _lib.check(lib.cgvae_gemm(form, _p(A), A.stride(0), _p(B), B.stride(0), _p(C), ldc, M, N, K, _p(bias), act, _p(Z),
                              _p(z_in), dact, _p(add), _p(ws), _SPLITK_WS_BYTES if ws is not None else 0, _p(tk),
                              _N_TICKETS if tk is not None else 0, st), "gemm")
    if t0 is not None:
        meta = dict(form=form, M=M, N=N, K=K, lda=A.stride(0), ldb=B.stride(0))
        if TIMER.keep_operands:
            meta.update(A=A, B=B, bias=bias, act=act, z_in=z_in, dact=dact, add=add)
        TIMER.end("gemm", t0, meta)
    return (C, Z) if z_out else C


def linear_fwd(x, W, b, act=0, save_pre=False):
    M, K = x.shape
    N = W.shape[0]
    return gemm(GEMM_NT, x, W, M, N, K, bias=b, act=act, z_out=save_pre)


def linear_pair_fwd(x, W1, W2):
    M, K = x.shape
    N1, N2 = W1.shape[0], W2.shape[0]
    adjacent = (W1.is_contiguous() and W2.is_contiguous() and W1.shape[1] == K and W2.shape[1] == K
                and W2.data_ptr() == W1.data_ptr() + 4 * W1.numel())
    if not adjacent:
        return linear_fwd(x, W1, None, 0), linear_fwd(x, W2, None, 0)
    _need_cuda(x, W1)
    lib = _lib.load()
    C1 = torch.empty((M, N1), dtype=torch.float32, device=x.device)
    C2 = torch.empty((M, N2), dtype=torch.float32, device=x.device)
    _lib.check(lib.cgvae_dense_pair_fwd(_p(x), x.stride(0), _p(W1), K, M, N1, N2, K, _p(C1), _p(C2), _stream()), "dense_pair_fwd")
    return C1, C2


def linear_bwd_input(gy, W, z_in=None, dact=0, add=None):
    M, N = gy.shape
    K = W.shape[1]
    return gemm(GEMM_NN, gy, W, M, K, N, z_in=z_in, dact=dact, add=add)


DEFER_MAX_ROWS = 128
_DEFERRED = None


def deferring(rows):
    return _DEFERRED is not None and rows <= DEFER_MAX_ROWS


WGRAD_PROBLEMS_PER_LAUNCH = 48


class DeferredGrads(object):

    def __init__(self, flush=True):
        self.flush = flush
        self.pending = []

    def __enter__(self):
        global _DEFERRED
        if _DEFERRED is not None:
            raise RuntimeError("DeferredGrads scopes do not nest")
        _DEFERRED = []
        return self

    def flush_now(self):
        global _DEFERRED
        pending, _DEFERRED = _DEFERRED, []
        if pending:
            wgrad_grouped(merge_deferred(pending))

    def __exit__(self, exc_type, exc, tb):
        global _DEFERRED
        pending, _DEFERRED = _DEFERRED, None
        if exc_type is None:
            self.pending = merge_deferred(pending)
            if self.flush:
                wgrad_grouped(self.pending)
        return False


_WGRAD_DTYPE = None


def _wgrad_dtype():
    global _WGRAD_DTYPE
    if _WGRAD_DTYPE is None:
        import numpy as np
        _WGRAD_DTYPE = np.dtype([("gy", np.uint64), ("x", np.uint64), ("dW", np.uint64), ("db", np.uint64),
                                 ("rows", np.int32), ("n_out", np.int32), ("n_in", np.int32), ("ldg", np.int32),
                                 ("ldx", np.int32), ("seg_rows", np.int32), ("seg_stride_g", np.int64),
                                 ("seg_stride_x", np.int64)], align=True)
        assert _WGRAD_DTYPE.itemsize == 72
    return _WGRAD_DTYPE


def wgrad_table(problems):
    import numpy as np
    table = np.zeros(len(problems), dtype=_wgrad_dtype())
    for i, (gy, x, dW, db) in enumerate(problems):
        _need_cuda(gy)
        if gy.stride(1) != 1 or (x is not None and x.stride(1) != 1):
            raise ValueError("wgrad_grouped: operands must have unit column stride")
        if dW is not None and not dW.is_contiguous():
            raise ValueError("wgrad_grouped: dW must be contiguous")
        table[i] = (gy.data_ptr(), x.data_ptr() if x is not None else 0, dW.data_ptr() if dW is not None else 0,
                    db.data_ptr() if db is not None else 0, gy.shape[0], gy.shape[1], x.shape[1] if x is not None else 0,
                    gy.stride(0), x.stride(0) if x is not None else 0, 0, 0, 0)
    return table


def wgrad_grouped_table(table, out_floats=0, keep=None):
    if len(table) == 0:
        return
    lib = _lib.load()
    t0 = TIMER.begin("wgrad_grouped") if TIMER is not None else None
    _lib.check(lib.cgvae_wgrad_grouped(table.ctypes.data, len(table), _stream()), "wgrad_grouped")
    if t0 is not None:
        TIMER.end("wgrad_grouped", t0, dict(problems=len(table), table=(keep if TIMER.keep_operands else None),
                                           out_floats=out_floats))


def wgrad_grouped(problems):
    if not problems:
        return
    out_floats = sum((p[2].numel() if p[2] is not None else 0) + (p[3].numel() if p[3] is not None else 0) for p in problems)
    wgrad_grouped_table(wgrad_table(problems), out_floats, list(problems))


def merge_deferred(pending):
    merged, by_gy = [], {}
    for gy, x, dW, db in pending:
        key = (gy.data_ptr(), gy.shape[0], gy.shape[1], gy.stride(0))
        hit = by_gy.get(key)
        if hit is not None and ((db is not None and merged[hit][3] is None and dW is None)
                                or (dW is not None and merged[hit][2] is None and db is None)):
            g0, x0, w0, b0 = merged[hit]
            merged[hit] = (g0, x if x0 is None else x0, dW if w0 is None else w0, db if b0 is None else b0)
            continue
        by_gy[key] = len(merged)
        merged.append((gy, x, dW, db))
    return merged


def flush_deferred(pending):
    wgrad_grouped(merge_deferred(pending))


def linear_bwd_weight(gy, x, param=None, shape=None):
    rows, n_out = gy.shape
    n_in = x.shape[1]
    if shape is not None and tuple(shape) != (n_out, n_in):
        raise ValueError("linear_bwd_weight: shape %s does not match gy^T x = (%d, %d)" % (tuple(shape), n_out, n_in))
    out = _grad_out(param, (n_out, n_in)) if param is not None else None
    if deferring(rows) and _has_sink(param) and gy.is_cuda and gy.stride(1) == 1 and x.stride(1) == 1:
        _DEFERRED.append((gy, x, out.detach(), None))
        return out
    return gemm(GEMM_TN, gy, x, n_out, n_in, rows, out=out)


def colsum(X, param=None):
    _need_cuda(X)
    M, N = X.shape
    if X.dtype != torch.float32 or (N > 1 and X.stride(1) != 1):
        raise RuntimeError("colsum: X must be float32 with unit inner stride (got %s %s)" % (X.dtype, tuple(X.stride())))
    lib = _lib.load()
    out = _grad_out(param, (N,)) if param is not None else torch.empty(N, dtype=torch.float32, device=X.device)
    if deferring(M) and _has_sink(param) and X.stride(1) == 1:
        _DEFERRED.append((X, None, None, out.detach()))
        return out
    _lib.check(lib.cgvae_colsum(_p(X), X.stride(0), M, N, _p(out), _stream()), "colsum")
    return out



class MessageTiles(object):

    def __init__(self, rc, bptr, ngroups, rec, n_batches_cap, n_edges):
        self.rc, self.bptr, self.ngroups, self.rec = int(rc), bptr, ngroups, rec
        self.n_batches_cap, self.n_edges = int(n_batches_cap), int(n_edges)
        self.fill = None


import os as _os
MSG_TC = _os.environ.get("CGVAE_MSG_TC", "auto")
MSG_TC_RC = int(_os.environ.get("CGVAE_MSG_TC_RC", "8"))
MSG_TC_CROSS_RC = int(_os.environ.get("CGVAE_MSG_TC_CROSS_RC", "8"))
MSG_TC_MIN_EDGES = 4096
MSG_TC_MIN_DEGREE = 12.0
MSG_TC_MIN_FILL = float(_os.environ.get("CGVAE_MSG_TC_MIN_FILL", "0.40"))
_TC_DECISIONS = {}


def message_tiles(geom, transposed=False, rc=None):
    rc = int(rc or MSG_TC_RC)
    cache = geom.__dict__.setdefault("_tiles", {})
    key = (rc, bool(transposed))
    hit = cache.get(key)
    if hit is not None:
        return hit
    lib = _lib.load()
    g = geom.graph
    if transposed:
        rowptr, col, slot_map, n_rows, n_part = g.rowptr_t, g.col_t, g.perm_t, g.n_send, g.n_recv
    else:
        rowptr, col, slot_map, n_rows, n_part = g.rowptr, g.col, None, g.n_recv, g.n_send
    dev = geom.basis.device
    n_chunks = (n_rows + rc - 1) // rc
    cap = int(lib.cgvae_msg_tiles_batches_cap(n_rows, n_part, g.n_edges, rc))
    rec_bytes = int(lib.cgvae_msg_tiles_rec_bytes())
    nbatch = torch.empty(max(n_chunks, 1), dtype=torch.int32, device=dev)
    bptr = torch.empty(n_chunks + 1, dtype=torch.int32, device=dev)
    ngroups = torch.empty(max(n_chunks, 1), dtype=torch.int32, device=dev)
    rec = torch.empty(cap * rec_bytes, dtype=torch.uint8, device=dev)
    _lib.check(lib.cgvae_msg_tiles_build(_p(rowptr), _p(col), _p(slot_map), n_rows, n_part, g.n_edges, _p(geom.basis),
                                         _p(geom.unit), geom.rb, rc, _p(nbatch), _p(bptr), _p(ngroups), _p(rec), cap, _stream()),
               "msg_tiles_build")
    tiles = MessageTiles(rc, bptr, ngroups, rec, cap, g.n_edges)
    cache[key] = tiles
    return tiles


def _tc_applies(geom, n_split):
    if MSG_TC == "0":
        return False
    g = geom.graph
    if g.n_recv != g.n_send or g.n_recv == 0 or geom.n_rbf > 15 or g.n_recv > 262144:
        return False
    if MSG_TC == "1":
        return True
    if n_split not in (3, 4):
        return False
    if g.n_edges < MSG_TC_MIN_EDGES or g.n_edges < MSG_TC_MIN_DEGREE * g.n_recv:
        return False
    key = (g.n_recv, (g.n_edges // g.n_recv) // 4, MSG_TC_RC)
    hit = _TC_DECISIONS.get(key)
    if hit is None:
        if torch.cuda.is_current_stream_capturing():
            return True
        tiles = message_tiles(geom, False)
        if tiles.fill is None:
            live_edges = int(g.rowptr[-1].item())
            n_batches = int(tiles.bptr[-1].item())
            tiles.fill = live_edges / max(1.0, 64.0 * n_batches)
        hit = tiles.fill >= MSG_TC_MIN_FILL
        _TC_DECISIONS[key] = hit
    return hit


def message_tc_fwd(n_split, phi, v_send, v_recv, geom, Wf, bf, res_s, res_v, want_q=False):
    lib = _lib.load()
    g = geom.graph
    F = phi.shape[-1]
    dev = phi.device
    rc = MSG_TC_RC if n_split == 3 else min(MSG_TC_RC, MSG_TC_CROSS_RC)
    tiles = message_tiles(geom, False, rc)
    out_s = torch.empty((g.n_recv, F), dtype=torch.float32, device=dev)
    out_v = torch.empty((g.n_recv, 3, F), dtype=torch.float32, device=dev)
    q = torch.empty((g.n_recv, 3, F), dtype=torch.float32, device=dev) if (want_q and n_split == 4) else None
    ws_bytes = int(lib.cgvae_message_tc_ws_bytes(n_split, tiles.rc, g.n_recv, F))
    ws = torch.empty(ws_bytes, dtype=torch.uint8, device=dev)
    t0 = TIMER.begin("message_fwd") if TIMER is not None else None
    _lib.check(lib.cgvae_message_tc_fwd(n_split, _p(phi), _p(v_send), _p(v_recv), _p(tiles.bptr), _p(tiles.ngroups), _p(tiles.rec),
                                        tiles.n_batches_cap, tiles.rc, _p(Wf), _p(bf), g.n_recv, F, geom.n_rbf, _p(res_s),
                                        _p(res_v), int(v_send is None), _p(out_s), _p(out_v), _p(q), _p(ws), ws_bytes, _stream()),
               "message_tc_fwd")
    if t0 is not None:
        TIMER.end("message_fwd", t0, dict(n_split=n_split, E=g.n_edges, n_recv=g.n_recv, n_send=g.n_send, F=F,
                                          R=geom.n_rbf, v_zero=v_send is None, tc=True))
    return out_s, out_v, q


def message_fwd(n_split, phi, v_send, v_recv, geom, Wf, bf, res_s, res_v, want_q=False):
    _need_cuda(phi)
    if _tc_applies(geom, n_split):
        return message_tc_fwd(n_split, phi, v_send, v_recv, geom, Wf, bf, res_s, res_v, want_q)
    lib = _lib.load()
    g = geom.graph
    F = phi.shape[-1]
    dev = phi.device
    out_s = torch.empty((g.n_recv, F), dtype=torch.float32, device=dev)
    out_v = torch.empty((g.n_recv, 3, F), dtype=torch.float32, device=dev)
    q = torch.empty((g.n_recv, 3, F), dtype=torch.float32, device=dev) if (want_q and n_split == 4) else None
    t0 = TIMER.begin("message_fwd") if TIMER is not None else None
    _lib.check(lib.cgvae_message_fwd(n_split, _p(phi), _p(v_send), _p(v_recv), _p(g.rowptr), _p(g.col), _p(geom.basis),
                                     _p(geom.unit), _p(Wf), _p(bf), g.n_recv, g.n_send, F, geom.n_rbf, geom.rb, _p(res_s),
                                     _p(res_v), int(v_send is None), _p(out_s), _p(out_v), _p(q), _stream()), "message_fwd")
    if t0 is not None:
        TIMER.end("message_fwd", t0, dict(n_split=n_split, E=g.n_edges, n_recv=g.n_recv, n_send=g.n_send, F=F,
                                          R=geom.n_rbf, v_zero=v_send is None))
    return out_s, out_v, q


def message_bwd(n_split, phi, v_send, v_recv, q, geom, Wf, bf, g_out_s, g_out_v, residual, sink=True):
    _need_cuda(phi)
    lib = _lib.load()
    g = geom.graph
    F = phi.shape[-1]
    dev = phi.device
    g_phi = torch.empty((g.n_send, n_split, F), dtype=torch.float32, device=dev)
    g_v = torch.empty((g.n_send, 3, F), dtype=torch.float32, device=dev)
    dWf = _grad_out(Wf, (n_split * F, geom.n_rbf)) if sink else torch.empty((n_split * F, geom.n_rbf), dtype=torch.float32, device=dev)
    dbf = _grad_out(bf, (n_split * F,)) if sink else torch.empty((n_split * F,), dtype=torch.float32, device=dev)
    ws_bytes = int(lib.cgvae_message_bwd_ws_bytes(n_split, F, geom.rb, g.n_send))
    ws = torch.empty(ws_bytes, dtype=torch.uint8, device=dev)
    t0 = TIMER.begin("message_bwd") if TIMER is not None else None
    _lib.check(lib.cgvae_message_bwd(n_split, _p(phi), _p(v_send), _p(v_recv), _p(q), _p(g.rowptr_t), _p(g.col_t), _p(g.perm_t),
                                     _p(geom.basis), _p(geom.unit), _p(Wf), _p(bf), g.n_recv, g.n_send, F, geom.n_rbf, geom.rb,
                                     _p(g_out_s), _p(g_out_v), int(bool(residual)), int(v_send is None), _p(g_phi), _p(g_v),
                                     _p(dWf), _p(dbf), _p(ws), ws_bytes, _stream()), "message_bwd")
    if t0 is not None:
        TIMER.end("message_bwd", t0, dict(n_split=n_split, E=g.n_edges, n_recv=g.n_recv, n_send=g.n_send, F=F,
                                          R=geom.n_rbf, v_zero=v_send is None))
    return g_phi, g_v, dWf, dbf


def message9_fwd(phi, s, sbar, v, vbar, geom, Wf, bf, residual):
    _need_cuda(phi)
    lib = _lib.load()
    g = geom.graph
    n, F = s.shape
    outs = [torch.empty_like(s), torch.empty_like(sbar), torch.empty_like(v), torch.empty_like(vbar)]
    _lib.check(lib.cgvae_message9_fwd(_p(phi), _p(s), _p(sbar), _p(v), _p(vbar), _p(g.rowptr), _p(g.col), _p(geom.basis),
                                      _p(geom.unit), _p(Wf), _p(bf), n, F, geom.n_rbf, geom.rb, int(bool(residual)),
                                      _p(outs[0]), _p(outs[1]), _p(outs[2]), _p(outs[3]), _stream()), "message9_fwd")
    return outs


def message9_bwd(phi, s, sbar, v, vbar, geom, Wf, bf, residual, g_s, g_sbar, g_v, g_vbar):
    _need_cuda(phi)
    lib = _lib.load()
    g = geom.graph
    n, F = s.shape
    dev = s.device
    gi = [torch.empty_like(s), torch.empty_like(sbar), torch.empty_like(v), torch.empty_like(vbar)]
    g_phi = torch.empty((n, 9, F), dtype=torch.float32, device=dev)
    gw = torch.empty((g.n_edges, 9 * F), dtype=torch.float32, device=dev)
    _lib.check(lib.cgvae_message9_bwd(_p(phi), _p(s), _p(sbar), _p(v), _p(vbar), _p(g.rowptr), _p(g.col), _p(g.rowptr_t),
                                      _p(g.col_t), _p(g.perm_t), _p(geom.basis), _p(geom.unit), _p(Wf), _p(bf), n, g.n_edges, F,
                                      geom.n_rbf, geom.rb, int(bool(residual)), _p(g_s), _p(g_sbar), _p(g_v), _p(g_vbar), _p(gi[0]),
                                      _p(gi[1]), _p(gi[2]), _p(gi[3]), _p(g_phi), _p(gw), _stream()), "message9_bwd")
    R = geom.n_rbf
    E = g.n_edges
    if E > 0 and deferring(E):
        dWf = linear_bwd_weight(gw, geom.basis[:, :R], Wf)
        dbf = linear_bwd_weight(gw, geom.basis[:, R:R + 1], bf).reshape(9 * F)
    elif E > 0:
        fork = Fork(dev)
        with fork.branch():
            dWf = gemm(GEMM_TN, gw, geom.basis, 9 * F, R, E, out=_grad_out(Wf, (9 * F, R)))
            dbf = gemm(GEMM_TN, gw, geom.basis[:, R:], 9 * F, 1, E, out=_grad_out(bf, (9 * F,)).view(9 * F, 1)).reshape(9 * F)
        if deferring(n):
            fork.join()
    else:
        dWf = torch.zeros((9 * F, R), dtype=torch.float32, device=dev)
        dbf = torch.zeros((9 * F,), dtype=torch.float32, device=dev)
    return gi[0], gi[1], gi[2], gi[3], g_phi, dWf, dbf



def update_norm_fwd(s, Vv):
    _need_cuda(s)
    lib = _lib.load()
    N, F = s.shape
    x = torch.empty((N, 2 * F), dtype=torch.float32, device=s.device)
    _lib.check(lib.cgvae_update_norm_fwd(_p(s), _p(Vv), N, F, _p(x), _stream()), "update_norm_fwd")
    return x


def update_combine_fwd(s, v, Uv, Vv, q, residual):
    _need_cuda(Uv)
    lib = _lib.load()
    N, _, F = Uv.shape
    s_out = torch.empty((N, F), dtype=torch.float32, device=Uv.device)
    v_out = torch.empty((N, 3, F), dtype=torch.float32, device=Uv.device)
    _lib.check(lib.cgvae_update_combine_fwd(_p(s), _p(v), _p(Uv), _p(Vv), _p(q), N, F, int(bool(residual)), _p(s_out), _p(v_out),
                                            _stream()), "update_combine_fwd")
    return s_out, v_out


def update_combine_bwd(Uv, Vv, q, g_s, g_v, cat=False):
    _need_cuda(Uv)
    lib = _lib.load()
    N, _, F = Uv.shape
    gq = torch.empty_like(q)
    if cat:
        gUV = torch.empty((N, 3, 2 * F), dtype=torch.float32, device=Uv.device)
        gUv, gVv = gUV[:, :, :F], gUV[:, :, F:]
        _lib.check(lib.cgvae_update_combine_bwd_ld(_p(Uv), _p(Vv), _p(q), _p(g_s), _p(g_v), N, F, _p(gq), _p(gUV), gUV.data_ptr() + 4 * F,
                                                   2 * F, _stream()), "update_combine_bwd_ld")
        return gq, gUv, gVv
    gUv = torch.empty_like(Uv)
    gVv = torch.empty_like(Vv)
    _lib.check(lib.cgvae_update_combine_bwd(_p(Uv), _p(Vv), _p(q), _p(g_s), _p(g_v), N, F, _p(gq), _p(gUv), _p(gVv), _stream()),
               "update_combine_bwd")
    return gq, gUv, gVv


def update_norm_bwd(x, Vv, gx, g_s, gVv, residual):
    _need_cuda(x)
    lib = _lib.load()
    N, _, F = Vv.shape
    gs_in = torch.empty((N, F), dtype=torch.float32, device=x.device)
    if not gVv.is_contiguous():
        _lib.check(lib.cgvae_update_norm_bwd_ld(_p(x), _p(Vv), _p(gx), _p(g_s), N, F, int(bool(residual)), _p(gs_in), _p(gVv),
                                                gVv.stride(1), _stream()), "update_norm_bwd_ld")
        return gs_in
    _lib.check(lib.cgvae_update_norm_bwd(_p(x), _p(Vv), _p(gx), _p(g_s), N, F, int(bool(residual)), _p(gs_in), _p(gVv), _stream()),
               "update_norm_bwd")
    return gs_in


def segment_reduce_fwd(X, seg, mean, param=None):
    _need_cuda(X)
    lib = _lib.load()
    X = _f32(X)
    W = int(np.prod(X.shape[1:]))
    shape = (seg.n_beads,) + tuple(X.shape[1:])
    out = _grad_out(param, shape) if param is not None else torch.empty(shape, dtype=torch.float32, device=X.device)
    _lib.check(lib.cgvae_segment_reduce_fwd(_p(X), _p(seg.rowptr), _p(seg.atoms), seg.n_beads, W, int(bool(mean)), _p(out),
                                            _stream()), "segment_reduce_fwd")
    return out


def segment_reduce_bwd(g_out, seg, mean):
    _need_cuda(g_out)
    lib = _lib.load()
    g_out = _f32(g_out)
    W = int(np.prod(g_out.shape[1:]))
    g_X = torch.empty((seg.n,) + tuple(g_out.shape[1:]), dtype=torch.float32, device=g_out.device)
    _lib.check(lib.cgvae_segment_reduce_bwd(_p(g_out), _p(seg.mapping), _p(seg.rowptr), seg.n, W, int(bool(mean)), _p(g_X),
                                            _stream()), "segment_reduce_bwd")
    return g_X


def gather_rows(table, idx):
    _need_cuda(table, idx)
    lib = _lib.load()
    idx = idx.to(torch.int64).contiguous()
    W = table.shape[1]
    out = torch.empty((idx.shape[0], W), dtype=torch.float32, device=table.device)
    error_flags(table.device)
    _lib.check(lib.cgvae_gather_rows(_p(table), _p(idx), idx.shape[0], W, table.shape[0], _p(out), _stream()), "gather_rows")
    return out


def lift_fwd(V, cg_xyz, seg, mode, pin):
    _need_cuda(V, cg_xyz)
    lib = _lib.load()
    F = V.shape[-1]
    out = torch.empty((seg.n, 3), dtype=torch.float32, device=V.device)
    error_flags(V.device)
    _lib.check(lib.cgvae_lift_fwd(_p(V), _p(_f32(cg_xyz)), _p(seg.mapping), _p(seg.rank), _p(seg.rowptr), _p(seg.atoms), _p(pin),
                                  seg.n, seg.n_beads, F, mode, _p(out), _stream()), "lift_fwd")
    return out


def lift_bwd(g_xyz, seg, F, mode, pin):
    _need_cuda(g_xyz)
    lib = _lib.load()
    g_V = torch.empty((seg.n_beads, 3, F), dtype=torch.float32, device=g_xyz.device)
    _lib.check(lib.cgvae_lift_bwd(_p(_f32(g_xyz)), _p(seg.mapping), _p(seg.rank), _p(seg.rowptr), _p(seg.atoms), _p(pin), seg.n,
                                  seg.n_beads, F, mode, _p(g_V), _stream()), "lift_bwd")
    return g_V


def vec_to_planar(v_nf3):
    _need_cuda(v_nf3)
    lib = _lib.load()
    v_nf3 = _f32(v_nf3)
    N, F, _ = v_nf3.shape
    out = torch.empty((N, 3, F), dtype=torch.float32, device=v_nf3.device)
    _lib.check(lib.cgvae_vec_to_planar(_p(v_nf3), N, F, _p(out), _stream()), "vec_to_planar")
    return out


def vec_from_planar(v_n3f):
    _need_cuda(v_n3f)
    lib = _lib.load()
    v_n3f = _f32(v_n3f)
    N, _, F = v_n3f.shape
    out = torch.empty((N, F, 3), dtype=torch.float32, device=v_n3f.device)
    _lib.check(lib.cgvae_vec_from_planar(_p(v_n3f), N, F, _p(out), _stream()), "vec_from_planar")
    return out


def adam_clip_step(p, g, m, v, step, max_norm, lr, betas=(0.9, 0.999), eps=1e-8, norm_out=None, grad_scale=1.0,
                   loss=None, loss_scale=1.0, loss_limit=float("inf"), skipped=None):
    _need_cuda(p, g, m, v, step)
    lib = _lib.load()
    ws_bytes = int(lib.cgvae_adam_ws_bytes())
    ws = torch.empty(ws_bytes, dtype=torch.uint8, device=p.device)
    t0 = TIMER.begin("adam_clip") if TIMER is not None else None
    _lib.check(lib.cgvae_adam_clip_step(_p(p), _p(g), _p(m), _p(v), p.numel(), float(max_norm), float(grad_scale), float(lr), float(betas[0]),
                                        float(betas[1]), float(eps), _p(step), _p(norm_out), _p(loss), float(loss_scale),
                                        float(min(loss_limit, 3.0e38)), _p(skipped), _p(ws), ws_bytes, _stream()),
               "adam_clip_step")
    if t0 is not None:
        TIMER.end("adam_clip", t0, dict(n=p.numel()))


def set_pdl(on):
    return bool(_lib.load().cgvae_set_pdl(int(bool(on))))


MATMUL_PRECISIONS = ("highest", "high")


def set_matmul_precision(mode):
    if mode not in MATMUL_PRECISIONS:
        raise ValueError("matmul precision must be one of %s, got %r" % (MATMUL_PRECISIONS, mode))
    rc = _lib.load().cgvae_set_matmul_precision(MATMUL_PRECISIONS.index(mode))
    if rc < 0:
        _lib.check(rc, "set_matmul_precision")
    return MATMUL_PRECISIONS[rc]


def get_matmul_precision():
    return MATMUL_PRECISIONS[_lib.load().cgvae_get_matmul_precision()]


@_contextlib.contextmanager
def matmul_precision(mode):
    prev = set_matmul_precision(mode)
    try:
        yield
    finally:
        set_matmul_precision(prev)


def register_const_range(t):
    lib = _lib.load()
    if t is None:
        _lib.check(lib.cgvae_register_const_range(None, 0), "register_const_range")
    else:
        _lib.check(lib.cgvae_register_const_range(_p(t), t.numel() * t.element_size()), "register_const_range")


def register_const_params(module):
    for p in module.parameters():
        if p.is_cuda:
            register_const_range(p.data)


def adam_ws(device):
    lib = _lib.load()
    return torch.zeros(int(lib.cgvae_adam_ws_bytes()) // 4, dtype=torch.float32, device=device)


def grad_sumsq(g, loss, ws):
    _need_cuda(g, ws)
    lib = _lib.load()
    _lib.check(lib.cgvae_grad_sumsq(_p(g), g.numel(), _p(loss), _p(ws), ws.numel() * 4, _stream()), "grad_sumsq")


def adam_apply(p, g, m, v, step, max_norm, lr, ws, betas=(0.9, 0.999), eps=1e-8, grad_scale=1.0, use_ws_loss=False, loss_scale=1.0,
               loss_limit=float("inf"), skipped=None):
    _need_cuda(p, g, m, v, step, ws)
    lib = _lib.load()
    _lib.check(lib.cgvae_adam_apply(_p(p), _p(g), _p(m), _p(v), p.numel(), float(max_norm), float(grad_scale), float(lr), float(betas[0]),
                                    float(betas[1]), float(eps), _p(step), None, int(bool(use_ws_loss)), float(loss_scale),
                                    float(min(loss_limit, 3.0e38)), _p(skipped), _p(ws), ws.numel() * 4, _stream()), "adam_apply")



def fill(shape, value, like):
    lib = _lib.load()
    _f32(like)
    out = torch.empty(shape, dtype=torch.float32, device=like.device)
    _need_cuda(out)
    _lib.check(lib.cgvae_fill(_p(out), out.numel(), float(value), _stream()), "fill")
    return out


def vae_latent_fwd(mu, logvar, eps):
    _need_cuda(logvar)
    lib = _lib.load()
    logvar = _f32(logvar)
    sigma = torch.empty_like(logvar)
    z = torch.empty_like(logvar) if eps is not None else None
    _lib.check(lib.cgvae_vae_latent_fwd(_p(_f32(mu)) if eps is not None else None, _p(logvar), _p(_f32(eps)) if eps is not None else None,
                                        logvar.numel(), _p(sigma), _p(z), _stream()), "vae_latent_fwd")
    return z, sigma


def vae_latent_bwd(g_z, g_sigma, eps, sigma):
    lib = _lib.load()
    g_mu = torch.empty_like(sigma) if g_z is not None else None
    g_logvar = torch.empty_like(sigma)
    _lib.check(lib.cgvae_vae_latent_bwd(_p(g_z), _p(g_sigma), _p(eps), _p(sigma), sigma.numel(), _p(g_mu), _p(g_logvar), _stream()),
               "vae_latent_bwd")
    return g_mu, g_logvar


def std_logvar_fwd(x, c):
    _need_cuda(x)
    lib = _lib.load()
    x = _f32(x)
    y = torch.empty_like(x)
    _lib.check(lib.cgvae_std_logvar_fwd(_p(x), x.numel(), float(c), _p(y), _stream()), "std_logvar_fwd")
    return y


def std_logvar_bwd(gy, y, c):
    lib = _lib.load()
    gx = torch.empty_like(y)
    _lib.check(lib.cgvae_std_logvar_bwd(_p(_f32(gy)), _p(y), y.numel(), float(c), _p(gx), _stream()), "std_logvar_bwd")
    return gx


def loss_fwd(xyz, xyz_rec, bond_graph, mu, sigma, pmu, pstd, norms, beta, gamma, out=None):
    _need_cuda(xyz_rec)
    lib = _lib.load()
    dev = xyz_rec.device
    out4 = out if out is not None else torch.empty(4, dtype=torch.float32, device=dev)
    ws_bytes = int(lib.cgvae_loss_ws_bytes())
    ws = torch.empty(ws_bytes, dtype=torch.uint8, device=dev)
    n_beads, F = (mu.shape[0], mu.shape[1]) if mu is not None else (0, 0)
    _lib.check(lib.cgvae_loss_fwd(_p(xyz), _p(xyz_rec), xyz_rec.shape[0], _p(bond_graph.rowptr) if bond_graph is not None else None,
                                  _p(bond_graph.col) if bond_graph is not None else None, _p(mu), _p(sigma), _p(pmu), _p(pstd),
                                  n_beads, F, _p(norms), float(beta), float(gamma), _p(out4), _p(ws), ws_bytes, _stream()), "loss_fwd")
    return out4


def loss_bwd(g_loss, xyz, xyz_rec, bond_graph, mu, sigma, pmu, pstd, norms, beta, gamma):
    lib = _lib.load()
    g_rec = torch.empty_like(xyz_rec)
    g_mu = torch.empty_like(mu) if mu is not None else None
    g_sigma = torch.empty_like(mu) if mu is not None else None
    g_pmu = torch.empty_like(pmu) if pmu is not None else None
    g_pstd = torch.empty_like(pmu) if pmu is not None else None
    n_beads, F = (mu.shape[0], mu.shape[1]) if mu is not None else (0, 0)
    _lib.check(lib.cgvae_loss_bwd(_p(g_loss), _p(xyz), _p(xyz_rec), xyz_rec.shape[0], _p(bond_graph.rowptr) if bond_graph is not None else None,
                                  _p(bond_graph.col) if bond_graph is not None else None, _p(mu), _p(sigma), _p(pmu), _p(pstd), n_beads,
                                  F, _p(norms), float(beta), float(gamma), _p(g_rec), _p(g_mu), _p(g_sigma), _p(g_pmu), _p(g_pstd),
                                  _stream()), "loss_bwd")
    return g_rec, g_mu, g_sigma, g_pmu, g_pstd


def pin_mask(idx, n_atoms, count=None):
    _need_cuda(idx)
    lib = _lib.load()
    idx = idx.to(torch.int64).contiguous()
    nbytes = (n_atoms + 3) // 4 * 4
    buf = torch.empty(max(nbytes, 4), dtype=torch.uint8, device=idx.device)
    error_flags(idx.device)
    _lib.check(lib.cgvae_pin_mask(_p(idx), idx.numel(), _p(count), n_atoms, _p(buf), buf.numel(), _stream()), "pin_mask")
    return buf[:n_atoms]


def dihedral_loss_fwd(xyz, xyz_rec, idx, count=None, norm=None):
    _need_cuda(xyz_rec)
    lib = _lib.load()
    idx = idx.to(torch.int64).contiguous()
    D = idx.shape[0]
    dev = xyz_rec.device
    contrib = torch.empty((D, 4, 3), dtype=torch.float32, device=dev)
    out = torch.empty(1, dtype=torch.float32, device=dev)
    ws = torch.empty(256, dtype=torch.float32, device=dev)
    _lib.check(lib.cgvae_dihedral_loss_fwd(_p(_f32(xyz)), _p(_f32(xyz_rec)), _p(idx), D, _p(count), _p(norm), _p(contrib), _p(out),
                                           _p(ws), 1024, _stream()), "dihedral_loss_fwd")
    return out, contrib


def dihedral_loss_bwd(g_loss, contrib, graph, n_atoms, count=None, norm=None):
    lib = _lib.load()
    g = torch.empty((n_atoms, 3), dtype=torch.float32, device=contrib.device)
    _lib.check(lib.cgvae_dihedral_loss_bwd(_p(g_loss), _p(contrib), _p(graph.rowptr), _p(graph.col), n_atoms, contrib.shape[0],
                                           _p(count), _p(norm), _p(g), _stream()), "dihedral_loss_bwd")
    return g
```

include/cgvae_b200.h:

```cpp
#ifndef CGVAE_B200_H_
#define CGVAE_B200_H_

#include <stddef.h>
#include <stdint.h>

#ifdef __cplusplus
extern "C" {
#endif

typedef void* cgvae_stream_t;

#define CGVAE_ABI_VERSION 1

enum { CGVAE_ACT_NONE = 0, CGVAE_ACT_SWISH = 1, CGVAE_ACT_RELU = 2, CGVAE_ACT_TANH = 3,
       CGVAE_ACT_SIGMOID = 4, CGVAE_ACT_SHIFTED_SOFTPLUS = 5, CGVAE_ACT_LEAKY_RELU = 6, CGVAE_ACT_ELU = 7 };
enum { CGVAE_GEMM_NT = 0,
       CGVAE_GEMM_NN = 1,
       CGVAE_GEMM_TN = 2   };

int cgvae_abi_version(void);
const char* cgvae_last_error(void);
unsigned long long cgvae_launch_count(void);
enum { CGVAE_ERR_LIFT_RANK_BIT = 1,
       CGVAE_ERR_EMBED_INDEX_BIT = 2,
       CGVAE_ERR_BEAD_INDEX_BIT = 4,
       CGVAE_ERR_NODE_INDEX_BIT = 8    };
int cgvae_set_error_flags(int device, int32_t* flags);


size_t cgvae_radius_graph_ws_bytes(int64_t n, int64_t n_frames);
int cgvae_radius_graph_count(const float* xyz, int64_t n, const int64_t* frame_ptr, int64_t n_frames,
                             float cutoff, int undirected, int use_cells, int32_t* deg, void* ws,
                             size_t ws_bytes, cgvae_stream_t stream);
int cgvae_radius_graph_fill(const float* xyz, int64_t n, const int64_t* frame_ptr, int64_t n_frames,
                            float cutoff, int undirected, int use_cells, const int64_t* rowptr,
                            int64_t* out_pairs, void* ws, size_t ws_bytes, cgvae_stream_t stream);

int cgvae_exclusive_scan(const int32_t* counts, int64_t n, int64_t* out, cgvae_stream_t stream);

int cgvae_edge_orientation(const int64_t* pairs, int64_t n_edges, int32_t* flags, cgvae_stream_t stream);

int cgvae_csr_count(const int64_t* pairs, int64_t n_edges, const int64_t* n_edges_dev, int symmetrize,
                    int64_t n_recv, int64_t n_send, int32_t* deg_r, int32_t* deg_s, cgvae_stream_t stream);
int cgvae_scan_i32(const int32_t* counts, int64_t n, int32_t* out, cgvae_stream_t stream);
int cgvae_csr_fill(const int64_t* pairs, int64_t n_edges, const int64_t* n_edges_dev, int symmetrize,
                   int64_t n_recv, int64_t n_send,
                   const int32_t* rowptr_r, const int32_t* rowptr_s, int32_t* scratch ,
                   int32_t* col, int32_t* eid, int32_t* col_t, int32_t* perm_t, cgvae_stream_t stream);

int cgvae_segment_count(const int64_t* mapping, int64_t n, int64_t n_beads, int32_t* deg, cgvae_stream_t stream);
int cgvae_segment_rank(const int64_t* mapping, int64_t n, int64_t n_beads, const int32_t* rowptr_b,
                       int32_t* scratch , int32_t* atoms, int32_t* slot_of_atom, int64_t* rank,
                       cgvae_stream_t stream);


int cgvae_edge_geometry(const float* xyz_send, const float* xyz_recv, const float* r_edge, const int32_t* rowptr,
                        const int32_t* col, int64_t n_recv, int64_t n_edges, const float* coef, int R, int RB, float cutoff,
                        const float* edge_wgt, const int32_t* eid, float* basis, float* unit,
                        cgvae_stream_t stream);


int cgvae_gemm(int form, const float* A, int64_t lda, const float* B, int64_t ldb, float* C, int64_t ldc,
               int64_t M, int64_t N, int64_t K, const float* bias, int act, float* z_out,
               const float* z_in, int dact, const float* add, void* ws, size_t ws_bytes,
               int32_t* counters, int n_counters, cgvae_stream_t stream);
int cgvae_dense_pair_fwd(const float* x, int64_t ldx, const float* W, int64_t ldw, int64_t M, int64_t N1, int64_t N2,
                         int64_t K, float* C1, float* C2, cgvae_stream_t stream);
int cgvae_colsum(const float* X, int64_t ldx, int64_t M, int64_t N, float* out, cgvae_stream_t stream);

typedef struct cgvae_wgrad_problem {
  const float* gy;
  const float* x;
  float* dW;
  float* db;
  int32_t rows, n_out, n_in, ldg, ldx, seg_rows;
  int64_t seg_stride_g, seg_stride_x;
} cgvae_wgrad_problem;
int cgvae_wgrad_grouped(const cgvae_wgrad_problem* problems, int n_problems, cgvae_stream_t stream);


int cgvae_message_fwd(int n_split, const float* phi, const float* v_send, const float* v_recv,
                      const int32_t* rowptr, const int32_t* col, const float* basis, const float* unit,
                      const float* Wf, const float* bf, int64_t n_recv, int64_t n_send, int F, int R, int RB,
                      const float* res_s, const float* res_v, int v_is_zero,
                      float* out_s, float* out_v, float* q, cgvae_stream_t stream);

size_t cgvae_message_bwd_ws_bytes(int n_split, int F, int RB, int64_t n_send);
int cgvae_message_bwd(int n_split, const float* phi, const float* v_send, const float* v_recv, const float* q,
                      const int32_t* rowptr_t, const int32_t* col_t, const int32_t* perm_t,
                      const float* basis, const float* unit, const float* Wf, const float* bf,
                      int64_t n_recv, int64_t n_send, int F, int R, int RB,
                      const float* g_out_s, const float* g_out_v, int residual, int v_is_zero,
                      float* g_phi, float* g_v_send, float* dWf, float* dbf,
                      void* ws, size_t ws_bytes, cgvae_stream_t stream);

int64_t cgvae_msg_tiles_batches_cap(int64_t n_rows, int64_t n_partners, int64_t n_edge_slots, int RC);
size_t cgvae_msg_tiles_rec_bytes(void);
int cgvae_msg_tiles_build(const int32_t* rowptr, const int32_t* col, const int32_t* slot_map, int64_t n_rows,
                          int64_t n_partners, int64_t n_edge_slots, const float* basis, const float* unit, int RB, int RC,
                          int32_t* nbatch, int32_t* bptr, int32_t* ngroups, void* rec, int64_t n_batches_cap,
                          cgvae_stream_t stream);
size_t cgvae_message_tc_ws_bytes(int n_split, int RC, int64_t n_rows, int F);
int cgvae_message_tc_fwd(int n_split, const float* phi, const float* v_send, const float* v_recv, const int32_t* bptr,
                         const int32_t* ngroups, const void* rec, int64_t n_batches_cap, int RC, const float* Wf,
                         const float* bf, int64_t n_recv, int F, int R, const float* res_s, const float* res_v,
                         int v_is_zero, float* out_s, float* out_v, float* q, void* ws, size_t ws_bytes,
                         cgvae_stream_t stream);

int cgvae_message9_fwd(const float* phi, const float* s, const float* sbar, const float* v, const float* vbar,
                       const int32_t* rowptr, const int32_t* col, const float* basis, const float* unit,
                       const float* Wf, const float* bf, int64_t n, int F, int R, int RB, int residual,
                       float* out_s, float* out_sbar, float* out_v, float* out_vbar, cgvae_stream_t stream);
int cgvae_message9_bwd(const float* phi, const float* s, const float* sbar, const float* v, const float* vbar,
                       const int32_t* rowptr, const int32_t* col,
                       const int32_t* rowptr_t, const int32_t* col_t, const int32_t* perm_t,
                       const float* basis, const float* unit, const float* Wf, const float* bf,
                       int64_t n, int64_t n_edge_slots, int F, int R, int RB, int residual,
                       const float* g_s, const float* g_sbar, const float* g_v, const float* g_vbar,
                       float* gi_s, float* gi_sbar, float* gi_v, float* gi_vbar, float* g_phi, float* gw,
                       cgvae_stream_t stream);


int cgvae_update_norm_fwd(const float* s, const float* Vv, int64_t N, int F, float* x, cgvae_stream_t stream);
int cgvae_update_combine_fwd(const float* s, const float* v, const float* Uv, const float* Vv, const float* q,
                             int64_t N, int F, int residual, float* s_out, float* v_out, cgvae_stream_t stream);
int cgvae_update_combine_bwd(const float* Uv, const float* Vv, const float* q, const float* g_s, const float* g_v,
                             int64_t N, int F, float* gq, float* gUv, float* gVv, cgvae_stream_t stream);
int cgvae_update_norm_bwd(const float* x, const float* Vv, const float* gx, const float* g_s,
                          int64_t N, int F, int residual, float* gs_in, float* gVv, cgvae_stream_t stream);
int cgvae_update_combine_bwd_ld(const float* Uv, const float* Vv, const float* q, const float* g_s, const float* g_v, int64_t N, int F,
                                float* gq, float* gUv, float* gVv, int64_t ldg, cgvae_stream_t stream);
int cgvae_update_norm_bwd_ld(const float* x, const float* Vv, const float* gx, const float* g_s, int64_t N, int F, int residual,
                             float* gs_in, float* gVv, int64_t ldg, cgvae_stream_t stream);


int cgvae_segment_reduce_fwd(const float* X, const int32_t* rowptr_b, const int32_t* atoms, int64_t n_beads,
                             int64_t W, int mean, float* out, cgvae_stream_t stream);
int cgvae_segment_reduce_bwd(const float* g_out, const int64_t* mapping, const int32_t* rowptr_b, int64_t N,
                             int64_t W, int mean, float* g_X, cgvae_stream_t stream);
int cgvae_gather_rows(const float* table, const int64_t* idx, int64_t N, int64_t W, int64_t n_rows, float* out,
                      cgvae_stream_t stream);

int cgvae_lift_fwd(const float* V, const float* cg_xyz, const int64_t* mapping, const int64_t* rank,
                   const int32_t* rowptr_b, const int32_t* atoms, const uint8_t* pin, int64_t N, int64_t n_beads,
                   int F, int mode, float* xyz_out, cgvae_stream_t stream);
int cgvae_lift_bwd(const float* g_xyz, const int64_t* mapping, const int64_t* rank, const int32_t* rowptr_b,
                   const int32_t* atoms, const uint8_t* pin, int64_t N, int64_t n_beads, int F, int mode,
                   float* g_V, cgvae_stream_t stream);


size_t cgvae_adam_ws_bytes(void);
int cgvae_adam_clip_step(float* p, const float* g, float* m, float* v, int64_t n, float max_norm, float grad_scale,
                         float lr, float beta1, float beta2, float eps, float* step, float* norm_out,
                         const float* loss, float loss_scale, float loss_limit, float* skipped, void* ws,
                         size_t ws_bytes, cgvae_stream_t stream);
int cgvae_grad_sumsq(const float* g, int64_t n, const float* loss, void* ws, size_t ws_bytes, cgvae_stream_t stream);
int cgvae_adam_apply(float* p, const float* g, float* m, float* v, int64_t n, float max_norm, float grad_scale, float lr, float beta1,
                     float beta2, float eps, float* step, float* norm_out, int use_ws_loss, float loss_scale, float loss_limit,
                     float* skipped, void* ws, size_t ws_bytes, cgvae_stream_t stream);

int cgvae_vae_latent_fwd(const float* mu, const float* logvar, const float* eps, int64_t n, float* sigma, float* z,
                         cgvae_stream_t stream);
int cgvae_vae_latent_bwd(const float* g_z, const float* g_sigma, const float* eps, const float* sigma, int64_t n, float* g_mu,
                         float* g_logvar, cgvae_stream_t stream);
int cgvae_std_logvar_fwd(const float* x, int64_t n, float c, float* y, cgvae_stream_t stream);
int cgvae_std_logvar_bwd(const float* gy, const float* y, int64_t n, float c, float* gx, cgvae_stream_t stream);
size_t cgvae_loss_ws_bytes(void);
int cgvae_loss_fwd(const float* xyz, const float* xyz_rec, int64_t n_atoms, const int32_t* bond_rowptr, const int32_t* bond_col,
                   const float* mu, const float* sigma, const float* pmu, const float* pstd, int64_t n_beads, int F,
                   const float* norms, float beta, float gamma, float* out4, void* ws, size_t ws_bytes,
                   cgvae_stream_t stream);
int cgvae_loss_bwd(const float* g_loss, const float* xyz, const float* xyz_rec, int64_t n_atoms, const int32_t* bond_rowptr,
                   const int32_t* bond_col, const float* mu, const float* sigma, const float* pmu, const float* pstd,
                   int64_t n_beads, int F, const float* norms, float beta, float gamma, float* g_xyz_rec, float* g_mu,
                   float* g_sigma, float* g_pmu, float* g_pstd, cgvae_stream_t stream);
int cgvae_dihedral_loss_fwd(const float* xyz, const float* xyz_rec, const int64_t* idx, int64_t n_dihe, const int64_t* n_live,
                            const float* norm, float* contrib, float* out, void* ws, size_t ws_bytes, cgvae_stream_t stream);
int cgvae_dihedral_loss_bwd(const float* g_loss, const float* contrib, const int32_t* rowptr, const int32_t* col, int64_t n_atoms,
                            int64_t n_dihe, const int64_t* n_live, const float* norm, float* g_xyz_rec, cgvae_stream_t stream);
int cgvae_pin_mask(const int64_t* idx, int64_t n_idx, const int64_t* n_live, int64_t n_atoms, uint8_t* pin, size_t pin_bytes,
                   cgvae_stream_t stream);
int cgvae_bond_graph(const float* xyz, const float* radius, int64_t n, float scale, uint8_t* bond, cgvae_stream_t stream);
int cgvae_sample_quality(const float* ref_xyz, const float* samples, const float* radius, const uint8_t* heavy, int64_t n,
                         int64_t n_samples, float scale, int32_t* counts, float* rmsd, cgvae_stream_t stream);
int cgvae_set_pdl(int on);
int cgvae_set_matmul_precision(int mode);
int cgvae_get_matmul_precision(void);
int cgvae_register_const_range(const void* p, size_t bytes);
int cgvae_fill(float* p, int64_t n, float value, cgvae_stream_t stream);

int cgvae_vec_to_planar(const float* v_nf3, int64_t N, int F, float* v_n3f, cgvae_stream_t stream);
int cgvae_vec_from_planar(const float* v_n3f, int64_t N, int F, float* v_nf3, cgvae_stream_t stream);

#ifdef __cplusplus
}
#endif
#endif
```

Before: 758.1.

## Fuse update-block elementwise ops into streaming GEMM epilogues and prologues

Adds fusion modes to the small-M streaming GEMM kernels. The forward update norm and combine steps now run in the NT GEMM epilogue from a shared-memory tile, with W rows regrouped per CTA so each CTA holds matching feature channels. The backward combine-gradient computation runs inside the NN GEMM's G-load prologue, and the norm backward runs in the cluster-reduction epilogue. The aim is to cut separate elementwise kernel launches and intermediate global round-trips in the decoder update block, at the cost of more shared memory, single-CTA launch bounds and considerably more complex kernels.

Result: no change. 759.0 (median of 6 runs) (+0.1%).

```diff
diff --git a/coarsegrainingvae_b200/_lib.py b/coarsegrainingvae_b200/_lib.py
--- a/coarsegrainingvae_b200/_lib.py
+++ b/coarsegrainingvae_b200/_lib.py
@@ -7,6 +7,8 @@
 HEADER_PATH = os.path.join(_HERE, "..", "include", "cgvae_b200.h")
 
 _lib = None
+
+NOT_FUSED = -2
 
 _P = ctypes.c_void_p
 _I64 = ctypes.c_int64
@@ -54,6 +56,9 @@
     "cgvae_update_norm_bwd": (_INT, [_P, _P, _P, _P, _I64, _INT, _INT, _P, _P, _P]),
     "cgvae_update_combine_bwd_ld": (_INT, [_P, _P, _P, _P, _P, _I64, _INT, _P, _P, _P, _I64, _P]),
     "cgvae_update_norm_bwd_ld": (_INT, [_P, _P, _P, _P, _I64, _INT, _INT, _P, _P, _I64, _P]),
+    "cgvae_update_pair_norm_fwd": (_INT, [_P, _P, _I64, _INT, _P, _P, _P, _P, _P]),
+    "cgvae_update_q_combine_fwd": (_INT, [_P, _P, _P, _I64, _INT, _P, _P, _P, _P, _INT, _P, _P, _P, _P]),
+    "cgvae_update_bwd_fused": (_INT, [_P, _P, _P, _P, _P, _P, _P, _P, _INT, _P, _I64, _INT, _INT, _P, _P, _P, _P, _P]),
     "cgvae_segment_reduce_fwd": (_INT, [_P, _P, _P, _I64, _I64, _INT, _P, _P]),
     "cgvae_segment_reduce_bwd": (_INT, [_P, _P, _P, _I64, _I64, _INT, _P, _P]),
     "cgvae_gather_rows": (_INT, [_P, _P, _I64, _I64, _I64, _P, _P]),
diff --git a/coarsegrainingvae_b200/csrc/gemm_stream.cu b/coarsegrainingvae_b200/csrc/gemm_stream.cu
--- a/coarsegrainingvae_b200/csrc/gemm_stream.cu
+++ b/coarsegrainingvae_b200/csrc/gemm_stream.cu
@@ -1,4 +1,5 @@
 #include "common.cuh"
+#include "update_elem.cuh"
 #include <cooperative_groups.h>
 #include <cuda.h>
 #include <algorithm>
@@ -16,6 +17,30 @@
   float* C2;
   int n_split;
   int64_t ldc2;
+};
+
+enum StreamFuseMode {
+  FUSE_NONE = 0,
+  FUSE_NORM_FWD = 1,
+  FUSE_COMBINE_FWD = 2,
+  FUSE_GQ_BWD = 3,
+  FUSE_NORM_BWD = 4,
+};
+struct StreamFusion {
+  int mode;
+  int F;
+  int splits;
+  int residual;
+  const float* s;
+  const float* v;
+  const float* Uv;
+  const float* Vv;
+  const float* q;
+  const float* x;
+  const float* g_s;
+  const float* g_v;
+  float* out0;
+  float* out1;
 };
 
 __device__ __forceinline__ float stream_epilogue(const StreamEpilogue& ep, float v, int64_t m, int64_t n, int64_t ldc) {
@@ -102,18 +127,28 @@
 constexpr uint32_t kBulkPiece = 32768;
 
 template <int MR, int RW>
-__global__ void __launch_bounds__(MR > 16 ? 256 : 512) gemm_nt_stream_kernel(
+__global__ void __launch_bounds__(MR > 16 ? 256 : 512, 1) gemm_nt_stream_kernel(
     const float* __restrict__ X, int64_t ldx, const float* __restrict__ W, int64_t ldw, float* __restrict__ C, int64_t ldc,
-    int M, int N, int K, int rows_per_cta, StreamEpilogue ep, int w_const) {
+    int M, int N, int K, int rows_per_cta, StreamEpilogue ep, StreamFusion fz, int w_const) {
   if (!w_const) CGVAE_KERNEL_PROLOGUE();
   extern __shared__ __align__(128) float smem[];
   constexpr int NV = RW * MR;
   float* Xs = smem;
   float* Ws = smem + (size_t)MR * K;
-  uint64_t* bar = reinterpret_cast<uint64_t*>(Ws + (size_t)rows_per_cta * K);
+  float* Ts = Ws + (size_t)rows_per_cta * K;
+  uint64_t* bar = reinterpret_cast<uint64_t*>(Ts + (fz.mode != FUSE_NONE ? (size_t)MR * rows_per_cta : 0));
   const int tid = threadIdx.x, lane = tid & 31, warp = tid >> 5, nwarps = blockDim.x >> 5;
-  const int row0 = blockIdx.x * rows_per_cta;
-  const int rows = min(rows_per_cta, N - row0);
+  int row0, rows, nch = 0;
+  if (fz.splits > 0) {
+    const int base = fz.F / (int)gridDim.x, extra = fz.F % (int)gridDim.x, b = (int)blockIdx.x;
+    nch = base + (b < extra ? 1 : 0);
+    row0 = b * base + min(b, extra);
+    rows = fz.splits * nch;
+  } else {
+    row0 = blockIdx.x * rows_per_cta;
+    rows = min(rows_per_cta, N - row0);
+  }
+  auto wrow = [&](int r) { return nch > 0 ? (r / nch) * fz.F + row0 + r % nch : row0 + r; };
 
   if (tid == 0) {
     bar_init(bar, 1);
@@ -125,13 +160,18 @@
   if (warp == 0 && elect_lane()) {
     const uint32_t row_bytes = (uint32_t)K * 4u;
     bar_expect_tx(bar, (uint32_t)(M + rows) * row_bytes);
-    if (ldw == K) {
-      const char* src = reinterpret_cast<const char*>(W + (int64_t)row0 * ldw);
-      char* dst = reinterpret_cast<char*>(Ws);
-      for (uint32_t off = 0, total = (uint32_t)rows * row_bytes; off < total; off += kBulkPiece)
-        bulk_g2s(dst + off, src + off, min(kBulkPiece, total - off), bar);
-    } else {
-      for (int r = 0; r < rows; ++r) bulk_g2s(Ws + (size_t)r * K, W + (int64_t)(row0 + r) * ldw, row_bytes, bar);
+    const int nblk = nch > 0 ? fz.splits : 1, blk_rows = nch > 0 ? nch : rows;
+    for (int kb = 0; kb < nblk; ++kb) {
+      const int64_t wr0 = wrow(kb * blk_rows);
+      float* wdst = Ws + (size_t)kb * blk_rows * K;
+      if (ldw == K) {
+        const char* src = reinterpret_cast<const char*>(W + wr0 * ldw);
+        char* dst = reinterpret_cast<char*>(wdst);
+        for (uint32_t off = 0, total = (uint32_t)blk_rows * row_bytes; off < total; off += kBulkPiece)
+          bulk_g2s(dst + off, src + off, min(kBulkPiece, total - off), bar);
+      } else {
+        for (int r = 0; r < blk_rows; ++r) bulk_g2s(wdst + (size_t)r * K, W + (wr0 + r) * ldw, row_bytes, bar);
+      }
     }
     if (w_const) pdl_wait();
     if (ldx == K) {
@@ -182,12 +222,33 @@
       for (int i = 0; i < CNT; ++i) {
         const int idx = base + i;
         const int r = idx / MR, m = idx % MR;
-        const int n = row0 + t0 + r;
         if (m < M && t0 + r < rows) {
-          if (ep.C2 != nullptr && n >= ep.n_split) ep.C2[(int64_t)m * ep.ldc2 + (n - ep.n_split)] = acc[i];
-          else C[(int64_t)m * ldc + n] = stream_epilogue(ep, acc[i], m, n, ldc);
+          const int n = wrow(t0 + r);
+          float y = acc[i];
+          if (ep.C2 != nullptr && n >= ep.n_split) ep.C2[(int64_t)m * ep.ldc2 + (n - ep.n_split)] = y;
+          else C[(int64_t)m * ldc + n] = y = stream_epilogue(ep, y, m, n, ldc);
+          if (fz.mode != FUSE_NONE) Ts[m * rows_per_cta + t0 + r] = y;
         }
       }
+    }
+  }
+  if (fz.mode == FUSE_NONE) return;
+  __syncthreads();
+  const int F = fz.F;
+  if (fz.mode == FUSE_NORM_FWD) {
+    for (int o = tid; o < (M / 3) * rows; o += blockDim.x) {
+      const int i = o / rows, t = o - i * rows, n = row0 + t;
+      if (n < F) fz.out0[(int64_t)i * 2 * F + n] = fz.s[(int64_t)i * F + n];
+      else
+        fz.out0[(int64_t)i * 2 * F + n] = update_norm_elem(Ts[(3 * i) * rows_per_cta + t], Ts[(3 * i + 1) * rows_per_cta + t],
+                                                           Ts[(3 * i + 2) * rows_per_cta + t]);
+    }
+  } else if (fz.mode == FUSE_COMBINE_FWD) {
+    for (int o = tid; o < M * nch; o += blockDim.x) {
+      const int i = o / nch, j = o - i * nch, f = row0 + j;
+      const float* T = Ts + i * rows_per_cta;
+      update_combine_fwd_elem(fz.s, fz.v, fz.Uv, fz.Vv, (int64_t)i * 3 * F + f, (int64_t)i * F + f, F, fz.residual, T[j], T[nch + j],
+                              T[2 * nch + j], fz.out0, fz.out1);
     }
   }
 }
@@ -199,9 +260,9 @@
 template <> struct VecT<4> { using type = float4; };
 
 template <int MR, int VEC, int NW>
-__global__ void __launch_bounds__(NW * 32) gemm_nn_stream_kernel(
+__global__ void __launch_bounds__(NW * 32, 1) gemm_nn_stream_kernel(
     const __grid_constant__ CUtensorMap wmap, const float* __restrict__ G, int64_t ldg, float* __restrict__ C, int64_t ldc,
-    int M, int N, int K, int k_per_cta, int box_rows, StreamEpilogue ep, int w_const) {
+    int M, int N, int K, int k_per_cta, int box_rows, StreamEpilogue ep, StreamFusion fz, int w_const) {
   if (!w_const) CGVAE_KERNEL_PROLOGUE();
   namespace cg = cooperative_groups;
   using vec_t = typename VecT<VEC>::type;
@@ -233,11 +294,58 @@
     }
   }
   if (w_const) CGVAE_KERNEL_PROLOGUE();
-  for (int idx = tid; idx < MR * cnt; idx += NW * 32) {
-    const int m = idx / cnt, j = idx - m * cnt;
-    Gt[j * MR + m] = (m < M) ? __ldg(G + (int64_t)m * ldg + kbeg + j) : 0.f;
+  constexpr int GB = 4;
+  const int gtot = MR * cnt;
+  if (fz.mode == FUSE_GQ_BWD) {
+    const int F = fz.F;
+    for (int base = tid; base < gtot; base += GB * NW * 32) {
+      float gs[GB], u[GB][3], w[GB][3], gv[GB][3];
+      int c[GB];
+#pragma unroll
+      for (int e = 0; e < GB; ++e) {
+        const int idx = base + e * NW * 32, m = idx / cnt, j = idx - m * cnt;
+        const bool ok = idx < gtot && m < M;
+        const int k = kbeg + j;
+        c[e] = ok ? k / F : 3;
+        const int f = ok ? k - c[e] * F : 0;
+        const int64_t o = (ok ? (int64_t)m * 3 * F : 0) + f;
+        gs[e] = fz.g_s[(ok ? (int64_t)m * F : 0) + f];
+#pragma unroll
+        for (int cc = 0; cc < 3; ++cc) {
+          u[e][cc] = fz.Uv[o + (int64_t)cc * F];
+          w[e][cc] = fz.Vv[o + (int64_t)cc * F];
+          gv[e][cc] = fz.g_v[o + (int64_t)cc * F];
+        }
+      }
+#pragma unroll
+      for (int e = 0; e < GB; ++e) {
+        const int idx = base + e * NW * 32, m = idx / cnt, j = idx - m * cnt;
+        const CombineBwd r = update_combine_bwd_vals(u[e], w[e], gv[e], 0.f, 0.f, gs[e]);
+        const float g = c[e] == 0 ? r.gq[0] : (c[e] == 1 ? r.gq[1] : (c[e] == 2 ? gs[e] : 0.f));
+        if (idx < gtot) Gt[j * MR + m] = g;
+      }
+    }
+  } else {
+    for (int base = tid; base < gtot; base += GB * NW * 32) {
+      float g[GB];
+#pragma unroll
+      for (int u = 0; u < GB; ++u) {
+        const int idx = base + u * NW * 32, m = idx / cnt, j = idx - m * cnt;
+        g[u] = (idx < gtot && m < M) ? __ldg(G + (int64_t)m * ldg + kbeg + j) : 0.f;
+      }
+#pragma unroll
+      for (int u = 0; u < GB; ++u) {
+        const int idx = base + u * NW * 32, m = idx / cnt, j = idx - m * cnt;
+        if (idx < gtot) Gt[j * MR + m] = g[u];
+      }
+    }
   }
   __syncthreads();
+  if (fz.mode == FUSE_GQ_BWD && blockIdx.x == 0)
+    for (int idx = tid; idx < M * cnt; idx += NW * 32) {
+      const int m = idx / cnt, j = idx - m * cnt;
+      fz.out0[(int64_t)m * 3 * fz.F + kbeg + j] = Gt[j * MR + m];
+    }
 
   float acc[MR][VEC];
 #pragma unroll
@@ -283,14 +391,33 @@
   cg::cluster_group cluster = cg::this_cluster();
   cluster.sync();
   const int S = (int)cluster.num_blocks(), rank = (int)cluster.block_rank();
-  for (int o = tid; o < MR * COLS; o += NW * 32) {
-    const int m = o / COLS, c = o - m * COLS;
-    if (m % S != rank) continue;
+  const int my_rows = (MR - rank + S - 1) / S;
+  for (int t = tid; t < my_rows * COLS; t += NW * 32) {
+    const int m = rank + (t / COLS) * S, c = t % COLS, o = m * COLS + c;
     const int n = col0 + c;
     if (m < M && n < N) {
       float s = 0.f;
       for (int z = 0; z < S; ++z) s += *cluster.map_shared_rank(part + o, z);
-      C[(int64_t)m * ldc + n] = stream_epilogue(ep, s, m, n, ldc);
+      s = stream_epilogue(ep, s, m, n, ldc);
+      if (fz.mode != FUSE_NORM_BWD) {
+        C[(int64_t)m * ldc + n] = s;
+        continue;
+      }
+      const int F = fz.F;
+      if (n < F) {
+        fz.out0[(int64_t)m * F + n] = update_norm_bwd_gs(fz.residual, fz.g_s, (int64_t)m * F + n, s);
+      } else {
+        const int f = n - F;
+        const int64_t o = (int64_t)m * 3 * F + f;
+        const CombineBwd r = update_combine_bwd_elem(fz.Uv, fz.Vv, fz.g_v, o, F, fz.q[o], fz.q[o + F], fz.g_s[(int64_t)m * F + f]);
+        const float scale = s / fz.x[(int64_t)m * 2 * F + n];
+        float* gUV = fz.out1 + (int64_t)m * 3 * 2 * F + f;
+#pragma unroll
+        for (int c = 0; c < 3; ++c) {
+          gUV[(int64_t)c * 2 * F] = r.gUv[c];
+          gUV[(int64_t)c * 2 * F + F] = fmaf(scale, fz.Vv[o + (int64_t)c * F], r.gVv[c]);
+        }
+      }
     }
   }
   cluster.sync();
@@ -330,12 +457,21 @@
   return a >= it->begin && a + bytes <= it->end;
 }
 
+constexpr StreamFusion kNoFusion{};
+
 template <int MR, int RW>
 static bool launch_nt(const float* X, int64_t ldx, const float* W, int64_t ldw, float* C, int64_t ldc, int M, int N, int K,
-                      const StreamEpilogue& ep, cudaStream_t st) {
+                      const StreamEpilogue& ep, cudaStream_t st, const StreamFusion& fz = kNoFusion) {
   const int w_const = weights_are_constant(W, sizeof(float) * ((size_t)(N - 1) * (size_t)ldw + (size_t)K)) ? 1 : 0;
   int rpc = (int)ceil_div(ceil_div(N, kNumSM), RW) * RW;
-  const size_t smem = sizeof(float) * ((size_t)MR * K + (size_t)rpc * K) + 16;
+  int grid = (int)ceil_div(N, rpc);
+  if (fz.splits > 0) {
+    if (N != fz.splits * fz.F || sizeof(float) * ((size_t)MR * K + (size_t)rpc * K) + 16 > kMaxStreamSmem) return false;
+    grid = std::min(kNumSM, fz.F);
+    rpc = fz.splits * (int)ceil_div(fz.F, grid);
+  }
+  const size_t tile = fz.mode != FUSE_NONE ? (size_t)MR * rpc : 0;
+  const size_t smem = sizeof(float) * ((size_t)MR * K + (size_t)rpc * K + tile) + 16;
   if (smem > kMaxStreamSmem) return false;
   static size_t attr_bytes = 0;
   if (smem > attr_bytes) {
@@ -345,16 +481,16 @@
     }
     attr_bytes = kMaxStreamSmem;
   }
-  const int tasks = rpc / RW;
+  const int tasks = (int)ceil_div(rpc, RW);
   const int nwarps = tasks <= 2 ? 2 : (tasks <= 4 ? 4 : ((tasks <= 8 || MR > 16) ? 8 : 16));
-  launch_kernel(gemm_nt_stream_kernel<MR, RW>, dim3((unsigned)ceil_div(N, rpc)), dim3(nwarps * 32), smem, st, X, ldx, W, ldw, C, ldc, M,
-                N, K, rpc, ep, w_const);
+  launch_kernel(gemm_nt_stream_kernel<MR, RW>, dim3((unsigned)grid), dim3(nwarps * 32), smem, st, X, ldx, W, ldw, C, ldc, M, N, K,
+                rpc, ep, fz, w_const);
   return true;
 }
 
 template <int MR, int VEC, int NW>
 static bool launch_nn(const float* G, int64_t ldg, const float* W, int64_t ldw, float* C, int64_t ldc, int M, int N, int K,
-                      const StreamEpilogue& ep, cudaStream_t st) {
+                      const StreamEpilogue& ep, cudaStream_t st, const StreamFusion& fz = kNoFusion, bool launch = true) {
   const int w_const = weights_are_constant(W, sizeof(float) * ((size_t)(K - 1) * (size_t)ldw + (size_t)N)) ? 1 : 0;
   constexpr int COLS = 32 * VEC;
   EncodeTiledFn encode = encode_tiled_fn();
@@ -371,6 +507,7 @@
   const size_t wt_floats = (size_t)std::max(nbox * box_rows, NW * MR) * COLS;
   const size_t smem = sizeof(float) * (wt_floats + (size_t)MR * COLS + (size_t)k_per_cta * MR) + 8 * NN_MAXBOX;
   if (smem > kMaxStreamSmem) return false;
+  if (!launch) return true;
   CUtensorMap map;
   const cuuint64_t gdim[2] = {(cuuint64_t)N, (cuuint64_t)K};
   const cuuint64_t gstride[1] = {(cuuint64_t)ldw * 4};
@@ -401,15 +538,19 @@
   attr[1].val.programmaticStreamSerializationAllowed = 1;
   cfg.attrs = attr;
   cfg.numAttrs = pdl_enabled() ? 2 : 1;
-  (void)cudaLaunchKernelEx(&cfg, gemm_nn_stream_kernel<MR, VEC, NW>, map, G, ldg, C, ldc, M, N, K, k_per_cta, box_rows, ep, w_const);
+  (void)cudaLaunchKernelEx(&cfg, gemm_nn_stream_kernel<MR, VEC, NW>, map, G, ldg, C, ldc, M, N, K, k_per_cta, box_rows, ep, fz, w_const);
   return true;
+}
+
+static bool stream_enabled() {
+  static const bool enabled = [] { const char* e = getenv("CGVAE_STREAM_GEMM"); return !(e && e[0] == '0'); }();
+  return enabled;
 }
 
 int launch_gemm_stream(int form, const float* A, int64_t lda, const float* B, int64_t ldb, float* C, int64_t ldc, int64_t M,
                        int64_t N, int64_t K, const float* bias, int act, float* z_out, const float* z_in, int dact,
                        const float* add, cudaStream_t st) {
-  static const bool enabled = [] { const char* e = getenv("CGVAE_STREAM_GEMM"); return !(e && e[0] == '0'); }();
-  if (!enabled || M > 48 || M < 1 || form == CGVAE_GEMM_TN) return 0;
+  if (!stream_enabled() || M > 48 || M < 1 || form == CGVAE_GEMM_TN) return 0;
   if (N * K < 64 * 64 || N >= (1 << 24) || K >= (1 << 24)) return 0;
   const StreamEpilogue ep{bias, act, z_out, z_in, dact, add, nullptr, 0, 0};
   const int m = (int)M, n = (int)N, k = (int)K;
@@ -430,22 +571,106 @@
   return launch_nn<48, 2, 8>(A, lda, B, ldb, C, ldc, m, n, k, ep, st);
 }
 
-int launch_dense_pair_stream(const float* X, int64_t ldx, const float* W, int64_t ldw, float* C1, int64_t ldc1, float* C2,
-                             int64_t ldc2, int64_t M, int64_t N1, int64_t N2, int64_t K, cudaStream_t st) {
-  static const bool enabled = [] { const char* e = getenv("CGVAE_STREAM_GEMM"); return !(e && e[0] == '0'); }();
-  if (!enabled || M > 48 || M < 1 || N1 + N2 >= (1 << 24) || K >= (1 << 24)) return 0;
+static int pair_stream(const float* X, int64_t ldx, const float* W, int64_t ldw, float* C1, int64_t ldc1, float* C2, int64_t ldc2,
+                       int64_t M, int64_t N1, int64_t N2, int64_t K, cudaStream_t st, const StreamFusion& fz) {
+  if (!stream_enabled() || M > 48 || M < 1 || N1 + N2 >= (1 << 24) || K >= (1 << 24)) return 0;
   if (K % 4 != 0 || K < 128 || ldx % 4 != 0 || ldw % 4 != 0 || !aligned16(X) || !aligned16(W)) return 0;
   const StreamEpilogue ep{nullptr, 0, nullptr, nullptr, 0, nullptr, C2, (int)N1, ldc2};
   const int m = (int)M, n = (int)(N1 + N2), k = (int)K;
-  if (M <= 12) return launch_nt<12, 4>(X, ldx, W, ldw, C1, ldc1, m, n, k, ep, st);
-  if (M <= 16) return launch_nt<16, 4>(X, ldx, W, ldw, C1, ldc1, m, n, k, ep, st);
-  if (M <= 36) return launch_nt<36, 2>(X, ldx, W, ldw, C1, ldc1, m, n, k, ep, st);
-  return launch_nt<48, 2>(X, ldx, W, ldw, C1, ldc1, m, n, k, ep, st);
+  if (M <= 12) return launch_nt<12, 4>(X, ldx, W, ldw, C1, ldc1, m, n, k, ep, st, fz);
+  if (M <= 16) return launch_nt<16, 4>(X, ldx, W, ldw, C1, ldc1, m, n, k, ep, st, fz);
+  if (M <= 36) return launch_nt<36, 2>(X, ldx, W, ldw, C1, ldc1, m, n, k, ep, st, fz);
+  return launch_nt<48, 2>(X, ldx, W, ldw, C1, ldc1, m, n, k, ep, st, fz);
+}
+
+int launch_dense_pair_stream(const float* X, int64_t ldx, const float* W, int64_t ldw, float* C1, int64_t ldc1, float* C2,
+                             int64_t ldc2, int64_t M, int64_t N1, int64_t N2, int64_t K, cudaStream_t st) {
+  return pair_stream(X, ldx, W, ldw, C1, ldc1, C2, ldc2, M, N1, N2, K, st, kNoFusion);
+}
+
+static bool launch_nn12(const float* G, int64_t ldg, const float* W, int64_t ldw, float* C, int64_t ldc, int M, int N, int K,
+                        const StreamEpilogue& ep, const StreamFusion& fz, cudaStream_t st, bool launch) {
+  if (K < 64 || N < 64 || ldw % 4 != 0 || !aligned16(W)) return false;
+  const bool wide = ceil_div(N, 64) * 2 > kNumSM;
+  return wide ? launch_nn<12, 4, 16>(G, ldg, W, ldw, C, ldc, M, N, K, ep, st, fz, launch)
+              : launch_nn<12, 2, 16>(G, ldg, W, ldw, C, ldc, M, N, K, ep, st, fz, launch);
 }
 
 }
 
 extern "C" {
+
+int cgvae_update_pair_norm_fwd(const float* v2, const float* UV, int64_t N, int F, const float* s, float* Uv, float* Vv, float* x,
+                               cgvae_stream_t stream) {
+  using namespace cgvae;
+  CGVAE_REQUIRE(N >= 1 && F >= 1, "update_pair_norm_fwd: bad sizes");
+  CGVAE_REQUIRE(v2 && UV && s && Uv && Vv && x, "update_pair_norm_fwd: null pointer");
+  StreamFusion fz{};
+  fz.mode = FUSE_NORM_FWD;
+  fz.F = F;
+  fz.s = s;
+  fz.out0 = x;
+  if (!pair_stream(v2, F, UV, F, Uv, F, Vv, F, 3 * N, F, F, F, (cudaStream_t)stream, fz)) return CGVAE_NOT_FUSED;
+  return launched("update_pair_norm_fwd");
+}
+
+int cgvae_update_q_combine_fwd(const float* h, const float* A1, const float* c1, int64_t N, int F, const float* s, const float* v,
+                               const float* Uv, const float* Vv, int residual, float* q, float* s_out, float* v_out,
+                               cgvae_stream_t stream) {
+  using namespace cgvae;
+  CGVAE_REQUIRE(N >= 1 && F >= 1, "update_q_combine_fwd: bad sizes");
+  CGVAE_REQUIRE(h && A1 && c1 && Uv && Vv && q && s_out && v_out && (!residual || (s && v)), "update_q_combine_fwd: null pointer");
+  if (!stream_enabled() || N > 12 || F % 4 != 0 || F < 128 || !aligned16(h) || !aligned16(A1)) return CGVAE_NOT_FUSED;
+  const StreamEpilogue ep{c1, 0, nullptr, nullptr, 0, nullptr, nullptr, 0, 0};
+  StreamFusion fz{};
+  fz.mode = FUSE_COMBINE_FWD;
+  fz.F = F;
+  fz.splits = 3;
+  fz.residual = residual;
+  fz.s = s;
+  fz.v = v;
+  fz.Uv = Uv;
+  fz.Vv = Vv;
+  fz.out0 = s_out;
+  fz.out1 = v_out;
+  if (!launch_nt<12, 4>(h, F, A1, F, q, 3 * (int64_t)F, (int)N, 3 * F, F, ep, (cudaStream_t)stream, fz)) return CGVAE_NOT_FUSED;
+  return launched("update_q_combine_fwd");
+}
+
+int cgvae_update_bwd_fused(const float* Uv, const float* Vv, const float* q, const float* x, const float* g_s, const float* g_v,
+                           const float* A1, const float* z, int dact, const float* A0, int64_t N, int F, int residual, float* gq,
+                           float* gz, float* gs_in, float* gUV, cgvae_stream_t stream) {
+  using namespace cgvae;
+  CGVAE_REQUIRE(N >= 1 && F >= 1, "update_bwd_fused: bad sizes");
+  CGVAE_REQUIRE(Uv && Vv && q && x && g_s && g_v && A1 && z && A0 && gq && gz && gs_in && gUV, "update_bwd_fused: null pointer");
+  if (!stream_enabled() || N > 12) return CGVAE_NOT_FUSED;
+  cudaStream_t st = (cudaStream_t)stream;
+  const int m = (int)N;
+  const StreamEpilogue ep1{nullptr, 0, nullptr, z, dact, nullptr, nullptr, 0, 0};
+  const StreamEpilogue ep2{nullptr, 0, nullptr, nullptr, 0, nullptr, nullptr, 0, 0};
+  StreamFusion fz1{};
+  fz1.mode = FUSE_GQ_BWD;
+  fz1.F = F;
+  fz1.Uv = Uv;
+  fz1.Vv = Vv;
+  fz1.q = q;
+  fz1.g_s = g_s;
+  fz1.g_v = g_v;
+  fz1.out0 = gq;
+  StreamFusion fz2 = fz1;
+  fz2.mode = FUSE_NORM_BWD;
+  fz2.residual = residual;
+  fz2.x = x;
+  fz2.out0 = gs_in;
+  fz2.out1 = gUV;
+  if (!launch_nn12(nullptr, 3 * (int64_t)F, A1, F, gz, F, m, F, 3 * F, ep1, fz1, st, false) ||
+      !launch_nn12(gz, F, A0, 2 * (int64_t)F, nullptr, 2 * (int64_t)F, m, 2 * F, F, ep2, fz2, st, false))
+    return CGVAE_NOT_FUSED;
+  launch_nn12(nullptr, 3 * (int64_t)F, A1, F, gz, F, m, F, 3 * F, ep1, fz1, st, true);
+  if (int rc = launched("update_gq_bwd")) return rc;
+  launch_nn12(gz, F, A0, 2 * (int64_t)F, nullptr, 2 * (int64_t)F, m, 2 * F, F, ep2, fz2, st, true);
+  return launched("update_norm_bwd_fused");
+}
 
 int cgvae_register_const_range(const void* p, size_t bytes) {
   using namespace cgvae;
diff --git a/coarsegrainingvae_b200/csrc/nodewise.cu b/coarsegrainingvae_b200/csrc/nodewise.cu
--- a/coarsegrainingvae_b200/csrc/nodewise.cu
+++ b/coarsegrainingvae_b200/csrc/nodewise.cu
@@ -1,4 +1,5 @@
 #include "common.cuh"
+#include "update_elem.cuh"
 
 namespace cgvae {
 
@@ -10,11 +11,8 @@
   const int64_t n = idx / F;
   const int f = (int)(idx % F);
   const float* p = Vv + n * 3 * F + f;
-  const float a = __fadd_rn(__fmul_rn(p[0], p[0]), 1e-10f);
-  const float b = __fadd_rn(__fmul_rn(p[F], p[F]), 1e-10f);
-  const float c = __fadd_rn(__fmul_rn(p[2 * (int64_t)F], p[2 * (int64_t)F]), 1e-10f);
   x[n * 2 * F + f] = s[idx];
-  x[n * 2 * F + F + f] = __fsqrt_rn(__fadd_rn(__fadd_rn(a, b), c));
+  x[n * 2 * F + F + f] = update_norm_elem(p[0], p[F], p[2 * (int64_t)F]);
 }
 
 __global__ void __launch_bounds__(256) update_combine_fwd_kernel(const float* __restrict__ s, const float* __restrict__ v,
@@ -27,15 +25,7 @@
   const int64_t n = idx / F;
   const int f = (int)(idx % F);
   const int64_t o = n * 3 * F + f;
-  const float a_vv = q[o], a_sv = q[o + F], a_ss = q[o + 2 * (int64_t)F];
-  float inner = 0.f;
-#pragma unroll
-  for (int c = 0; c < 3; ++c) {
-    const float u = Uv[o + (int64_t)c * F], w = Vv[o + (int64_t)c * F];
-    inner = fmaf(u, w, inner);
-    v_out[o + (int64_t)c * F] = (residual ? v[o + (int64_t)c * F] : 0.f) + u * a_vv;
-  }
-  s_out[idx] = (residual ? s[idx] : 0.f) + (inner * a_sv + a_ss);
+  update_combine_fwd_elem(s, v, Uv, Vv, o, idx, F, residual, q[o], q[o + F], q[o + 2 * (int64_t)F], s_out, v_out);
 }
 
 __global__ void __launch_bounds__(256) update_combine_bwd_kernel(const float* __restrict__ Uv, const float* __restrict__ Vv,
@@ -50,21 +40,14 @@
   const int f = (int)(idx % F);
   const int64_t o = n * 3 * F + f;
   const int64_t og = n * 3 * ldg + f;
-  const float a_vv = q[o], a_sv = q[o + F];
-  const float gs = g_s[idx];
-  float inner = 0.f, g_avv = 0.f;
-  const float t = gs * a_sv;
+  const CombineBwd r = update_combine_bwd_elem(Uv, Vv, g_v, o, F, q[o], q[o + F], g_s[idx]);
 #pragma unroll
   for (int c = 0; c < 3; ++c) {
-    const float u = Uv[o + (int64_t)c * F], w = Vv[o + (int64_t)c * F], g = g_v[o + (int64_t)c * F];
-    inner = fmaf(u, w, inner);
-    g_avv = fmaf(g, u, g_avv);
-    gUv[og + (int64_t)c * ldg] = g * a_vv + t * w;
-    gVv[og + (int64_t)c * ldg] = t * u;
-  }
-  gq[o] = g_avv;
-  gq[o + F] = gs * inner;
-  gq[o + 2 * (int64_t)F] = gs;
+    gUv[og + (int64_t)c * ldg] = r.gUv[c];
+    gVv[og + (int64_t)c * ldg] = r.gVv[c];
+  }
+#pragma unroll
+  for (int c = 0; c < 3; ++c) gq[o + (int64_t)c * F] = r.gq[c];
 }
 
 __global__ void __launch_bounds__(256) update_norm_bwd_kernel(const float* __restrict__ x, const float* __restrict__ Vv,
@@ -76,7 +59,7 @@
   if (idx >= N * F) return;
   const int64_t n = idx / F;
   const int f = (int)(idx % F);
-  gs_in[idx] = (residual ? g_s[idx] : 0.f) + gx[n * 2 * F + f];
+  gs_in[idx] = update_norm_bwd_gs(residual, g_s, idx, gx[n * 2 * F + f]);
   const float scale = gx[n * 2 * F + F + f] / x[n * 2 * F + F + f];
   const int64_t o = n * 3 * F + f, og = n * 3 * ldg + f;
 #pragma unroll
diff --git a/coarsegrainingvae_b200/csrc/update_elem.cuh b/coarsegrainingvae_b200/csrc/update_elem.cuh
--- /dev/null
+++ b/coarsegrainingvae_b200/csrc/update_elem.cuh
@@ -0,0 +1,64 @@
+#pragma once
+
+namespace cgvae {
+
+__device__ __forceinline__ float update_norm_elem(float p0, float p1, float p2) {
+  const float a = __fadd_rn(__fmul_rn(p0, p0), 1e-10f);
+  const float b = __fadd_rn(__fmul_rn(p1, p1), 1e-10f);
+  const float c = __fadd_rn(__fmul_rn(p2, p2), 1e-10f);
+  return __fsqrt_rn(__fadd_rn(__fadd_rn(a, b), c));
+}
+
+__device__ __forceinline__ void update_combine_fwd_elem(const float* __restrict__ s, const float* __restrict__ v,
+                                                        const float* __restrict__ Uv, const float* __restrict__ Vv, int64_t o,
+                                                        int64_t idx, int F, int residual, float a_vv, float a_sv, float a_ss,
+                                                        float* __restrict__ s_out, float* __restrict__ v_out) {
+  float inner = 0.f;
+#pragma unroll
+  for (int c = 0; c < 3; ++c) {
+    const float u = Uv[o + (int64_t)c * F], w = Vv[o + (int64_t)c * F];
+    inner = fmaf(u, w, inner);
+    v_out[o + (int64_t)c * F] = (residual ? v[o + (int64_t)c * F] : 0.f) + u * a_vv;
+  }
+  s_out[idx] = (residual ? s[idx] : 0.f) + (inner * a_sv + a_ss);
+}
+
+struct CombineBwd {
+  float gq[3];
+  float gUv[3], gVv[3];
+};
+__device__ __forceinline__ CombineBwd update_combine_bwd_vals(const float* u, const float* w, const float* g, float a_vv, float a_sv,
+                                                              float gs) {
+  CombineBwd r;
+  float inner = 0.f, g_avv = 0.f;
+  const float t = gs * a_sv;
+#pragma unroll
+  for (int c = 0; c < 3; ++c) {
+    inner = fmaf(u[c], w[c], inner);
+    g_avv = fmaf(g[c], u[c], g_avv);
+    r.gUv[c] = g[c] * a_vv + t * w[c];
+    r.gVv[c] = t * u[c];
+  }
+  r.gq[0] = g_avv;
+  r.gq[1] = gs * inner;
+  r.gq[2] = gs;
+  return r;
+}
+__device__ __forceinline__ CombineBwd update_combine_bwd_elem(const float* __restrict__ Uv, const float* __restrict__ Vv,
+                                                              const float* __restrict__ g_v, int64_t o, int F, float a_vv,
+                                                              float a_sv, float gs) {
+  float u[3], w[3], g[3];
+#pragma unroll
+  for (int c = 0; c < 3; ++c) {
+    u[c] = Uv[o + (int64_t)c * F];
+    w[c] = Vv[o + (int64_t)c * F];
+    g[c] = g_v[o + (int64_t)c * F];
+  }
+  return update_combine_bwd_vals(u, w, g, a_vv, a_sv, gs);
+}
+
+__device__ __forceinline__ float update_norm_bwd_gs(int residual, const float* __restrict__ g_s, int64_t idx, float gx_s) {
+  return (residual ? g_s[idx] : 0.f) + gx_s;
+}
+
+}
diff --git a/coarsegrainingvae_b200/functions.py b/coarsegrainingvae_b200/functions.py
--- a/coarsegrainingvae_b200/functions.py
+++ b/coarsegrainingvae_b200/functions.py
@@ -133,6 +133,17 @@
         return None, None, None, gs, gi_sbar, gi_v, gi_vbar, gW1, gb1, gW2, gb2, dWf, dbf
 
 
+def _uv_pair(U, V):
+    return (U.is_cuda and U.is_contiguous() and V.is_contiguous() and U.shape == V.shape
+            and V.data_ptr() == U.data_ptr() + 4 * U.numel()
+            and U.untyped_storage().data_ptr() == V.untyped_storage().data_ptr())
+
+
+def _update_fusable(pair, A0, c0, A1, c1):
+    return (ops.decoder_fusion() and pair and A0.is_contiguous() and A1.is_contiguous() and c0 is not None
+            and c1 is not None and c1.is_contiguous())
+
+
 class UpdateBlockFn(Function):
 
     @staticmethod
@@ -140,12 +151,22 @@
         s, v = s.contiguous(), v.contiguous()
         N, F = s.shape
         v2 = v.view(3 * N, F)
-        Uv, Vv = ops.linear_pair_fwd(v2, U, V)
-        Uv, Vv = Uv.view(N, 3, F), Vv.view(N, 3, F)
-        x = ops.update_norm_fwd(s, Vv)
+        fuse = _update_fusable(_uv_pair(U, V), A0, c0, A1, c1)
+        r = ops.update_pair_norm_fwd(v2, U.as_strided((2 * F, U.shape[1]), (U.shape[1], 1)), s) if fuse else None
+        if r is None:
+            Uv, Vv = ops.linear_pair_fwd(v2, U, V)
+            Uv, Vv = Uv.view(N, 3, F), Vv.view(N, 3, F)
+            x = ops.update_norm_fwd(s, Vv)
+        else:
+            Uv, Vv, x = r
+            Uv, Vv = Uv.view(N, 3, F), Vv.view(N, 3, F)
         h, z = ops.linear_fwd(x, A0, c0, act, save_pre=True)
-        q = ops.linear_fwd(h, A1, c1, 0).view(N, 3, F)
-        s_out, v_out = ops.update_combine_fwd(s, v, Uv, Vv, q, residual)
+        r = ops.update_q_combine_fwd(h, A1, c1, s, v, Uv, Vv, residual) if fuse else None
+        if r is None:
+            q = ops.linear_fwd(h, A1, c1, 0).view(N, 3, F)
+            s_out, v_out = ops.update_combine_fwd(s, v, Uv, Vv, q, residual)
+        else:
+            q, s_out, v_out = r
         ctx.residual, ctx.act = residual, act
         ctx.save_for_backward(v, Uv, Vv, x, h, z, q, U, V, A0, c0, A1, c1)
         return s_out, v_out
@@ -156,12 +177,27 @@
         v, Uv, Vv, x, h, z, q, U, V, A0, c0, A1, c1 = ctx.saved_tensors
         g_s, g_v = g_s.contiguous(), g_v.contiguous()
         N, _, F = v.shape
-        pair = (U.is_cuda and U.is_contiguous() and V.is_contiguous() and U.shape == V.shape
-                and V.data_ptr() == U.data_ptr() + 4 * U.numel()
-                and U.untyped_storage().data_ptr() == V.untyped_storage().data_ptr())
+        pair = _uv_pair(U, V)
+        v2 = v.view(3 * N, F)
+        r = (ops.update_bwd_fused(Uv, Vv, q, x, g_s, g_v, A1, z, ctx.act, A0, ctx.residual)
+             if _update_fusable(pair, A0, c0, A1, c1) else None)
+        if r is not None:
+            gq2, gz, gs_in, gUV2 = r
+            fork = ops.Fork(g_s.device, enabled=not ops.deferring(3 * N))
+            with fork.branch():
+                gA1 = ops.linear_bwd_weight(gq2, h, A1)
+                gc1 = ops.colsum(gq2, c1)
+                gA0 = ops.linear_bwd_weight(gz, x, A0)
+                gc0 = ops.colsum(gz, c0)
+            UV = U.as_strided((2 * F, U.shape[1]), (U.shape[1], 1))
+            gv_in = ops.linear_bwd_input(gUV2, UV, add=g_v.view(3 * N, F) if ctx.residual else None).view(N, 3, F)
+            with fork.branch():
+                gUVw = ops.linear_bwd_weight(gUV2, v2, U, shape=(2 * F, U.shape[1]))
+                gU, gV = gUVw[:F], gUVw[F:]
+            fork.join()
+            return None, None, gs_in, gv_in, gU, gV, gA0, gc0, gA1, gc1
         gq, gUv, gVv = ops.update_combine_bwd(Uv, Vv, q, g_s, g_v, cat=pair)
         gq2 = gq.view(N, 3 * F)
-        v2 = v.view(3 * N, F)
         if pair:
             gUV2 = gUv.as_strided((3 * N, 2 * F), (2 * F, 1))
             gUv2, gVv2 = gUV2[:, :F], gUV2[:, F:]
diff --git a/coarsegrainingvae_b200/ops.py b/coarsegrainingvae_b200/ops.py
--- a/coarsegrainingvae_b200/ops.py
+++ b/coarsegrainingvae_b200/ops.py
@@ -748,6 +748,68 @@
 
 
 
+_DECODER_FUSION = True
+
+
+def set_decoder_fusion(on):
+    global _DECODER_FUSION
+    prev, _DECODER_FUSION = _DECODER_FUSION, bool(on)
+    return prev
+
+
+def decoder_fusion():
+    return _DECODER_FUSION
+
+
+def _fused(rc, what):
+    if rc == _lib.NOT_FUSED:
+        return False
+    _lib.check(rc, what)
+    return True
+
+
+def update_pair_norm_fwd(v2, UV, s):
+    _need_cuda(v2)
+    lib = _lib.load()
+    N, F = s.shape
+    Uv = torch.empty((3 * N, F), dtype=torch.float32, device=v2.device)
+    Vv = torch.empty((3 * N, F), dtype=torch.float32, device=v2.device)
+    x = torch.empty((N, 2 * F), dtype=torch.float32, device=v2.device)
+    if not _fused(lib.cgvae_update_pair_norm_fwd(_p(v2), _p(UV), N, F, _p(s), _p(Uv), _p(Vv), _p(x), _stream()),
+                  "update_pair_norm_fwd"):
+        return None
+    return Uv, Vv, x
+
+
+def update_q_combine_fwd(h, A1, c1, s, v, Uv, Vv, residual):
+    _need_cuda(h)
+    lib = _lib.load()
+    N, F = h.shape
+    q = torch.empty((N, 3, F), dtype=torch.float32, device=h.device)
+    s_out = torch.empty((N, F), dtype=torch.float32, device=h.device)
+    v_out = torch.empty((N, 3, F), dtype=torch.float32, device=h.device)
+    if not _fused(lib.cgvae_update_q_combine_fwd(_p(h), _p(A1), _p(c1), N, F, _p(s), _p(v), _p(Uv), _p(Vv), int(bool(residual)),
+                                                 _p(q), _p(s_out), _p(v_out), _stream()), "update_q_combine_fwd"):
+        return None
+    return q, s_out, v_out
+
+
+def update_bwd_fused(Uv, Vv, q, x, g_s, g_v, A1, z, dact, A0, residual):
+    _need_cuda(Uv)
+    lib = _lib.load()
+    N, _, F = Uv.shape
+    dev = Uv.device
+    gq = torch.empty((N, 3 * F), dtype=torch.float32, device=dev)
+    gz = torch.empty((N, F), dtype=torch.float32, device=dev)
+    gs_in = torch.empty((N, F), dtype=torch.float32, device=dev)
+    gUV = torch.empty((3 * N, 2 * F), dtype=torch.float32, device=dev)
+    if not _fused(lib.cgvae_update_bwd_fused(_p(Uv), _p(Vv), _p(q), _p(x), _p(g_s), _p(g_v), _p(A1), _p(z), dact, _p(A0), N, F,
+                                             int(bool(residual)), _p(gq), _p(gz), _p(gs_in), _p(gUV), _stream()),
+                  "update_bwd_fused"):
+        return None
+    return gq, gz, gs_in, gUV
+
+
 def update_norm_fwd(s, Vv):
     _need_cuda(s)
     lib = _lib.load()
diff --git a/include/cgvae_b200.h b/include/cgvae_b200.h
--- a/include/cgvae_b200.h
+++ b/include/cgvae_b200.h
@@ -132,6 +132,16 @@
                                 float* gq, float* gUv, float* gVv, int64_t ldg, cgvae_stream_t stream);
 int cgvae_update_norm_bwd_ld(const float* x, const float* Vv, const float* gx, const float* g_s, int64_t N, int F, int residual,
                              float* gs_in, float* gVv, int64_t ldg, cgvae_stream_t stream);
+
+#define CGVAE_NOT_FUSED (-2)
+int cgvae_update_pair_norm_fwd(const float* v2, const float* UV, int64_t N, int F, const float* s, float* Uv, float* Vv, float* x,
+                               cgvae_stream_t stream);
+int cgvae_update_q_combine_fwd(const float* h, const float* A1, const float* c1, int64_t N, int F, const float* s, const float* v,
+                               const float* Uv, const float* Vv, int residual, float* q, float* s_out, float* v_out,
+                               cgvae_stream_t stream);
+int cgvae_update_bwd_fused(const float* Uv, const float* Vv, const float* q, const float* x, const float* g_s, const float* g_v,
+                           const float* A1, const float* z, int dact, const float* A0, int64_t N, int F, int residual, float* gq,
+                           float* gz, float* gs_in, float* gUV, cgvae_stream_t stream);
 
 
 int cgvae_segment_reduce_fwd(const float* X, const int32_t* rowptr_b, const int32_t* atoms, int64_t n_beads,
```
